# modelscope/FunCodec

Measured on AMD Instinct MI355X. Metric: audio-seconds encoded+decoded per wall-sec, 16k-nq32ds640, higher is better.
Workload: dtype f32; 1 GPU; BASELINE.json configs[1]: encodec 16k-nq32ds640 (57.6M, synthetic seeded checkpoint), run_mod=inference (encode + 32-stage RVQ + decode), 16 x 10 s utterances per GPU in micro-batches of 16, n_q=32; utterances_per_gpu=16, samples_per_utterance=160000, micro_batch=16, global_utterances=16, ranks_seen=1, parallelism=single GPU

## Files before the change

funcodec_amd/_lib.py:

```python
from __future__ import annotations

import ctypes as C
import os

from . import build as _build

FC_MAX_RATIOS = 8
FC_ABI_VERSION = 7


class FcArch(C.Structure):
    _fields_ = [
        ("abi_version", C.c_int32), ("sample_rate", C.c_int32), ("audio_normalize", C.c_int32),
        ("n_filters", C.c_int32), ("dimension", C.c_int32), ("n_ratios", C.c_int32),
        ("ratios", C.c_int32 * FC_MAX_RATIOS),
        ("kernel_size", C.c_int32), ("last_kernel_size", C.c_int32), ("residual_kernel_size", C.c_int32),
        ("compress", C.c_int32), ("lstm_layers", C.c_int32), ("lstm_skip", C.c_int32),
        ("elu_alpha", C.c_float), ("gn_eps", C.c_float),
        ("codebook_size", C.c_int32), ("num_quantizers", C.c_int32),
        ("norm_type", C.c_int32), ("causal", C.c_int32), ("n_residual_layers", C.c_int32), ("dilation_base", C.c_int32),
        ("model_type", C.c_int32), ("input_channels", C.c_int32), ("n_fft", C.c_int32), ("stft_hop", C.c_int32),
        ("ratios_f", C.c_int32 * FC_MAX_RATIOS),
        ("enc_conv_group_ratio", C.c_int32), ("dec_conv_group_ratio", C.c_int32), ("dec_tr_conv_group_ratio", C.c_int32),
        ("codec_dim", C.c_int32), ("codec_range", C.c_float),
        ("q0_ds_ratio", C.c_int32),
        ("seq_model", C.c_int32), ("seq_heads", C.c_int32), ("seq_ff", C.c_int32),
    ]


class FcWork(C.Structure):
    _fields_ = [("total_flops", C.c_double), ("total_bytes", C.c_double), ("conv_flops", C.c_double),
                ("conv_bytes", C.c_double), ("lstm_flops", C.c_double), ("rvq_flops", C.c_double),
                ("conv_launches", C.c_int32), ("total_launches", C.c_int32)]


class FcProf(C.Structure):
    _fields_ = [("kernel", C.c_char * 64), ("total_ms", C.c_double), ("flops", C.c_double), ("bytes", C.c_double),
                ("launches", C.c_int32), ("reserved", C.c_int32)]


FC_PROF_CLASSES = 48


class FcLauraStack(C.Structure):
    _fields_ = [("idim", C.c_int32), ("d_model", C.c_int32), ("heads", C.c_int32), ("ff", C.c_int32), ("layers", C.c_int32),
                ("act", C.c_int32), ("embed_relu", C.c_int32), ("norm_style", C.c_int32)]


class FcLauraArch(C.Structure):
    _fields_ = [("abi_version", C.c_int32), ("input_size", C.c_int32), ("vocab_size", C.c_int32), ("codebook_size", C.c_int32),
                ("codebook_dim", C.c_int32), ("num_quantizers", C.c_int32), ("predict_nq", C.c_int32), ("pos_emb_split", C.c_int32),
                ("bidirectional_inputs", C.c_int32), ("max_positions", C.c_int32),
                ("text_encoder", FcLauraStack), ("codec_lm", FcLauraStack), ("codec_encoder", FcLauraStack)]


_P = C.c_void_p
SYMBOLS = {
    "fc_abi_version": (C.c_int, []),
    "fc_last_error": (C.c_char_p, []),
    "fc_engine_create": (C.c_int, [C.POINTER(FcArch), C.c_int, C.POINTER(_P)]),
    "fc_engine_destroy": (None, [_P]),
    "fc_engine_num_weights": (C.c_int, [_P]),
    "fc_engine_weight_info": (C.c_int, [_P, C.c_int, C.POINTER(C.c_char_p), C.POINTER(C.c_int64)]),
    "fc_engine_set_weight": (C.c_int, [_P, C.c_char_p, _P, C.POINTER(C.c_int64), C.c_int]),
    "fc_engine_finalize": (C.c_int, [_P]),
    "fc_engine_hop_length": (C.c_int, [_P]),
    "fc_engine_frames": (C.c_int, [_P, C.c_int]),
    "fc_engine_decoded_samples": (C.c_int, [_P, C.c_int]),
    "fc_engine_workspace_bytes": (C.c_size_t, [_P, C.c_int, C.c_int]),
    "fc_encode": (C.c_int, [_P, _P, C.c_int, C.c_int, C.c_int, _P, _P, _P, _P, _P, _P, C.c_size_t, _P]),
    "fc_decode_emb": (C.c_int, [_P, _P, _P, C.c_int, C.c_int, C.c_int, _P, _P, C.c_size_t, _P]),
    "fc_decode_codes": (C.c_int, [_P, _P, C.c_int, C.c_int, C.c_int, C.c_int, _P, _P, _P, C.c_size_t, _P]),
    "fc_encode_decode": (C.c_int, [_P, _P, C.c_int, C.c_int, C.c_int, C.c_int, _P, _P, _P, _P, _P, _P, C.c_size_t, _P]),
    "fc_ragged_workspace_bytes": (C.c_size_t, [_P, C.c_int, C.c_int]),
    "fc_encode_ragged": (C.c_int, [_P, _P, _P, C.c_int, C.c_int, C.c_int, _P, _P, _P, _P, _P, _P, C.c_size_t, _P]),
    "fc_decode_emb_ragged": (C.c_int, [_P, _P, _P, _P, C.c_int, C.c_int, C.c_int, _P, _P, C.c_size_t, _P]),
    "fc_decode_codes_ragged": (C.c_int, [_P, _P, _P, C.c_int, C.c_int, C.c_int, C.c_int, _P, _P, _P, C.c_size_t, _P]),
    "fc_encode_decode_ragged": (C.c_int, [_P, _P, _P, C.c_int, C.c_int, C.c_int, C.c_int, _P, _P, _P, _P, _P, _P, C.c_size_t, _P]),
    "fc_engine_set_row_nq": (C.c_int, [_P, _P, C.c_int, _P]),
    "fc_rvq_encode": (C.c_int, [_P, _P, C.c_int, C.c_int, _P, _P, _P, C.c_size_t, _P]),
    "fc_q0_source_frames": (C.c_int, [C.c_int, _P]),
    "fc_layer_forward": (C.c_int, [_P, C.c_char_p, _P, C.c_int, C.c_int, C.c_int, _P, _P, C.c_size_t, _P]),
    "fc_layer_forward_src": (C.c_int, [_P, C.c_char_p, _P, _P, _P, _P, _P, C.c_int, C.c_int, C.c_int, _P, _P, C.c_size_t, _P]),
    "fc_layer_out_len": (C.c_int, [_P, C.c_char_p, C.c_int]),
    "fc_layer2d_forward": (C.c_int, [_P, C.c_char_p, _P, _P, _P, _P, C.c_int, C.c_int, C.c_int, C.c_int, C.c_int, _P, _P, C.c_size_t, _P]),
    "fc_layer2d_out_shape": (C.c_int, [_P, C.c_char_p, C.c_int, C.c_int, C.c_int, C.c_int, C.POINTER(C.c_int64)]),
    "fc_freq_synthesis": (C.c_int, [_P, _P, _P, _P, C.c_int, C.c_int, C.c_int, C.c_int, C.c_int, _P, _P, _P, C.c_size_t, _P]),
    "fc_freq_synthesis_size": (C.c_int, [_P, C.c_int, C.c_int, C.c_int, C.c_int, C.c_int, C.POINTER(C.c_size_t)]),
    "fc_lstm_forward": (C.c_int, [_P, C.c_char_p, _P, C.c_int, C.c_int, _P, _P, C.c_size_t, _P]),
    "fc_seq_forward": (C.c_int, [_P, C.c_char_p, _P, C.c_int, C.c_int, _P, _P, C.c_size_t, _P]),
    "fc_resblock_forward": (C.c_int, [_P, C.c_char_p, _P, C.c_int, C.c_int, _P, _P, C.c_size_t, _P]),
    "fc_resblock_forward_src": (C.c_int, [_P, C.c_char_p, _P, _P, _P, _P, C.c_int, C.c_int, _P, _P, C.c_size_t, _P]),
    "fc_engine_work": (C.c_int, [_P, C.c_int, C.c_int, C.c_int, C.POINTER(FcWork)]),
    "fc_engine_profile": (C.c_int, [_P, C.c_int]),
    "fc_engine_profile_read": (C.c_int, [_P, C.POINTER(FcProf)]),
    "fc_debug_timeline": (C.c_int, [_P]),
    "fc_debug_conv_layout": (C.c_int, [C.c_int] * 7 + [_P, _P, C.c_size_t, _P, C.c_size_t]),
    "fc_debug_freq_features": (C.c_int, [_P, C.c_size_t, C.c_int]),
    "fc_codec_json_bound": (C.c_size_t, [C.c_int, C.c_int]),
    "fc_format_codec_json": (C.c_int, [_P, C.c_int, C.c_int, C.c_int, C.c_int, C.c_int, _P, C.c_size_t, C.POINTER(C.c_size_t)]),
    "fc_write_wav_pcm16": (C.c_int, [C.c_char_p, _P, C.c_int, C.c_int, C.c_int]),
    "fc_overlap_add": (C.c_int, [_P, _P, C.c_int, C.c_int, C.c_int, C.c_int, C.c_int, _P, _P]),
    "fc_engine_status": (C.c_int, [_P, C.POINTER(C.c_uint)]),
    "fc_stream_state_bytes": (C.c_size_t, [_P, C.c_int]),
    "fc_stream_create": (C.c_int, [_P, C.c_int, C.c_int, C.c_int, _P, C.c_size_t, C.POINTER(_P)]),
    "fc_stream_destroy": (None, [_P]),
    "fc_stream_min_first": (C.c_int, [_P, C.c_int]),
    "fc_stream_workspace_bytes": (C.c_size_t, [_P]),
    "fc_stream_reset": (C.c_int, [_P, _P, _P]),
    "fc_stream_encode": (C.c_int, [_P, _P, C.c_int, C.c_int, _P, _P, _P, C.POINTER(C.c_int), _P, C.c_size_t, _P]),
    "fc_stream_decode_codes": (C.c_int, [_P, _P, C.c_int, C.c_int, _P, _P, _P, C.c_size_t, _P]),
    "fc_stream_decode_emb": (C.c_int, [_P, _P, C.c_int, C.c_int, _P, _P, C.c_size_t, _P]),
    "fc_stream_lstm_forward": (C.c_int, [_P, C.c_int, _P, C.c_int, _P, _P, C.c_size_t, _P]),
    "fc_seqstream_state_bytes": (C.c_size_t, [_P, C.c_int, C.c_int]),
    "fc_seqstream_create": (C.c_int, [_P, C.c_int, C.c_int, C.c_int, C.c_int, _P, C.c_size_t, C.POINTER(_P)]),
    "fc_seqstream_forward": (C.c_int, [_P, C.c_int, _P, C.c_int, _P, _P, C.c_size_t, _P]),
    "fc_slots_state_bytes": (C.c_size_t, [_P, C.c_int]),
    "fc_slots_create": (C.c_int, [_P, C.c_int, C.c_int, C.c_int, _P, C.c_size_t, C.POINTER(_P)]),
    "fc_slots_destroy": (None, [_P]),
    "fc_slots_min_first": (C.c_int, [_P, C.c_int]),
    "fc_slots_workspace_bytes": (C.c_size_t, [_P]),
    "fc_slots_encode": (C.c_int, [_P, _P, C.c_int, _P, _P, _P, _P, _P, _P, _P, C.c_size_t, _P]),
    "fc_slots_decode_codes": (C.c_int, [_P, _P, C.c_int, _P, _P, C.c_int, _P, _P, _P, C.c_size_t, _P]),
    "fc_slots_decode_emb": (C.c_int, [_P, _P, C.c_int, _P, _P, C.c_int, _P, _P, C.c_size_t, _P]),
    "fc_slots_lstm_forward": (C.c_int, [_P, C.c_int, _P, C.c_int, _P, _P, _P, _P, C.c_size_t, _P]),
    "fc_seqslots_state_bytes": (C.c_size_t, [_P, C.c_int, C.c_int]),
    "fc_seqslots_create": (C.c_int, [_P, C.c_int, C.c_int, C.c_int, C.c_int, _P, C.c_size_t, C.POINTER(_P)]),
    "fc_seqslots_forward": (C.c_int, [_P, C.c_int, _P, C.c_int, _P, _P, _P, _P, C.c_size_t, _P]),
    "fc_graphstream_set": (C.c_int, [_P, C.c_int]),
    "fc_graphstream_enabled": (C.c_int, [_P]),
    "fc_graphstream_counts": (C.c_int, [_P, C.POINTER(C.c_int64)]),
    "fc_graphslots_set": (C.c_int, [_P, C.c_int]),
    "fc_graphslots_enabled": (C.c_int, [_P]),
    "fc_graphslots_counts": (C.c_int, [_P, C.POINTER(C.c_int64)]),
    "fc_laura_create": (C.c_int, [C.POINTER(FcLauraArch), C.c_int, C.POINTER(_P)]),
    "fc_laura_destroy": (None, [_P]),
    "fc_laura_num_weights": (C.c_int, [_P]),
    "fc_laura_weight_info": (C.c_int, [_P, C.c_int, C.POINTER(C.c_char_p), C.POINTER(C.c_int64)]),
    "fc_laura_set_weight": (C.c_int, [_P, C.c_char_p, _P, C.POINTER(C.c_int64), C.c_int]),
    "fc_laura_finalize": (C.c_int, [_P]),
    "fc_laura_workspace_bytes": (C.c_size_t, [_P, C.c_int, C.c_int, C.c_int, C.c_int]),
    "fc_laura_encode": (C.c_int, [_P, _P, _P, _P, C.c_int, C.c_int, _P, _P, C.c_size_t, _P]),
    "fc_laura_lm_logprobs": (C.c_int, [_P, _P, _P, C.c_int, C.c_int, _P, _P, C.c_int, _P, C.c_int, _P, C.c_size_t, _P]),
    "fc_laura_decode_codec": (C.c_int, [_P, _P, _P, C.c_int, C.c_int, _P, _P, C.c_int, C.c_int, C.c_int, C.c_int, C.c_float,
                                        C.c_uint64, _P, _P, _P, _P, _P, C.c_size_t, _P]),
    "fc_laura_codec_emb": (C.c_int, [_P, _P, _P, C.c_int, C.c_int, _P, C.c_int, _P, C.c_int, _P, _P, C.c_size_t, _P]),
    "fc_laura_linear": (C.c_int, [_P, C.c_char_p, _P, C.c_int, C.c_int, C.c_int, _P, _P, C.c_size_t, _P]),
    "fc_laura_debug_probe": (C.c_int, [_P, C.c_size_t, C.c_int, C.c_int, C.c_int]),
    "fc_laura_set_persistent_step": (C.c_int, [_P, C.c_int]),
    "fc_laura_persistent_step_fallbacks": (C.c_int, [_P]),
    "fc_laura_slots_state_bytes": (C.c_size_t, [_P, C.c_int, C.c_int, C.c_int]),
    "fc_laura_slots_create": (C.c_int, [_P, C.c_int, C.c_int, C.c_int, _P, C.c_size_t, C.POINTER(_P)]),
    "fc_laura_slots_destroy": (None, [_P]),
    "fc_laura_slots_workspace_bytes": (C.c_size_t, [_P, C.c_int, C.c_int]),
    "fc_laura_slots_start": (C.c_int, [_P, C.c_int, _P, C.c_int, _P, C.c_int, C.c_int, C.c_int, C.c_int, C.c_float, C.c_uint64, _P,
                                       _P, C.c_size_t, _P]),
    "fc_laura_slots_step": (C.c_int, [_P, C.c_int, _P, _P, _P]),
    "fc_laura_slots_take": (C.c_int, [_P, C.c_int, _P, C.c_int, _P, _P]),
    "fc_laura_slots_start_from": (C.c_int, [_P, C.c_int, C.c_int, C.c_int, C.c_int, C.c_int, C.c_float, C.c_uint64, _P, _P]),
    "fc_laura_slots_fork": (C.c_int, [_P, C.c_int, C.c_int, C.c_int, C.c_int, C.c_int, C.c_int, C.c_float, C.c_uint64, _P]),
    "fc_laura_slots_state_bytes_scored": (C.c_size_t, [_P, C.c_int, C.c_int, C.c_int, C.c_int]),
    "fc_laura_slots_create_scored": (C.c_int, [_P, C.c_int, C.c_int, C.c_int, C.c_int, _P, C.c_size_t, C.POINTER(_P)]),
    "fc_laura_slots_score": (C.c_int, [_P, C.c_int, _P, C.c_int, C.POINTER(C.c_int32), C.POINTER(C.c_int32)]),
    "fc_laura_slots_set_rules": (C.c_int, [_P, C.c_int, C.c_float, C.c_int, C.c_float, C.c_int, C.c_int]),
    "fc_laura_slots_start_many_workspace_bytes": (C.c_size_t, [_P, C.c_int, C.c_int, C.c_int]),
    "fc_laura_slots_start_many": (C.c_int, [_P, C.c_int, _P, _P, _P, C.c_int, _P, _P, C.c_int, _P, _P, _P, _P, _P, _P, C.c_size_t, _P]),
    "fc_laura_slots_start_from_session": (C.c_int, [_P, C.c_int, _P, C.c_int, C.c_int, C.c_int, C.c_int, C.c_float, C.c_uint64, _P, _P]),
    "fc_laura_slots_state_bytes_wide": (C.c_size_t, [_P, C.c_int, C.c_int, C.c_int, C.c_int]),
    "fc_laura_slots_create_wide": (C.c_int, [_P, C.c_int, C.c_int, C.c_int, C.c_int, _P, C.c_size_t, C.POINTER(_P)]),
    "fc_laura_slots_state_bytes_queued": (C.c_size_t, [_P, C.c_int, C.c_int, C.c_int, C.c_int]),
    "fc_laura_slots_create_queued": (C.c_int, [_P, C.c_int, C.c_int, C.c_int, C.c_int, _P, _P, C.c_size_t, C.POINTER(_P)]),
    "fc_laura_slots_submit": (C.c_int, [_P, C.c_int, C.c_int, C.c_int, C.c_int, C.c_float, C.c_uint64, C.c_float, C.c_int, C.c_float, C.c_int,
                                        C.c_int, C.POINTER(C.c_int32), _P]),
    "fc_laura_slots_queue_status": (C.c_int, [_P, C.POINTER(C.c_int64), C.POINTER(C.c_int64), C.POINTER(C.c_int64), C.POINTER(C.c_int64),
                                              C.POINTER(C.c_int64), _P]),
# ... 34 lines not shown
```

funcodec_amd/csrc/engine.hip:

```cpp
#include <hip/hip_runtime.h>

#include <algorithm>
#include <array>
#include <cmath>
#include <cstdio>
#include <cstring>
#include <map>
#include <memory>
#include <string>
#include <vector>

#include "../../include/funcodec_amd.h"
#include "kernels.h"
#include "laura_kernels.h"
#include "ragged_kernels.h"
#include "seq_kernels.h"
#include "slots_kernels.h"
#include "stream_kernels.h"

namespace {

thread_local std::string g_err;

int fail(const std::string& msg) { g_err = msg; return 1; }
// ... 40 lines not shown
    float *wt = nullptr, *bias = nullptr, *gamma = nullptr, *beta = nullptr;
    int* koff = nullptr;
};

struct LstmLayer {
    ConvLayer inproj;
    float* whh = nullptr;
    float* wcat = nullptr;
    float* bperm = nullptr;
};

struct LstmBlock {
    std::string prefix;
    int H = 0;
    std::vector<LstmLayer> layers;
};

struct TfLayer {
    ConvLayer qkv;
    ConvLayer out, ff1, ff2;
    float *n1g = nullptr, *n1b = nullptr, *n2g = nullptr, *n2b = nullptr;
};

struct TfBlock {
    std::string prefix;
    int C = 0, heads = 4, ff = 2048;
    std::vector<TfLayer> layers;
    float *ag = nullptr, *ab = nullptr;
};

struct Act {
    float* raw = nullptr;
    float* aff = nullptr;
    int C = 0, T = 0;
    bool normed = false;
    int ld = 0;
};

int ceil_div_i(int a, int b) { return (a + b - 1) / b; }

const char* kLstmPersistClass = "lstm_persist_kernel<NS> (whole recurrence of one SLSTM block, one launch)";
const char* kLstmWaveClass = "lstm_wave_kernel<NS> (whole recurrence of one SLSTM block: T + L - 1 launches incl. gaps)";
const char* kRvqClass = "rvq_encode_kernel<D, RS> (all stages of the residual quantiser)";

}

struct fc_engine {
    fc_arch arch;
    int device = 0;
    bool finalized = false;
    std::vector<std::pair<std::string, std::vector<int64_t>>> expected;
    std::map<std::string, HostTensor> host;
    ConvLayer enc_first, enc_last, dec_first, dec_last;
    struct ResBlock {
        ConvLayer shortcut, block1, block3;
        bool fused_head = false;
        float *wsc = nullptr, *wb1 = nullptr;
        float *bsc = nullptr, *bb1 = nullptr;
    };
    struct Stage { std::vector<ResBlock> res; ConvLayer resample; };
    std::vector<Stage> enc_stages, dec_stages;
    LstmBlock enc_lstm, dec_lstm;
    TfBlock enc_tf, dec_tf;
    std::map<std::string, TfBlock*> tf_by_prefix;
    std::map<std::string, ConvLayer*> by_prefix;
    std::map<std::string, ResBlock*> res_by_prefix;
    ConvLayer enc2_first, dec2_last, stft, istft;
    ConvLayer q_in, q_out;
    bool q_proj = false;
    int cdim() const { return q_proj ? arch.codec_dim : arch.dimension; }
    int audio_ch() const { return arch.model_type == 0 && arch.input_channels == 2 ? 2 : 1; }
    std::vector<std::vector<ConvLayer>> dec_up_phases;
    int halo2 = 3;
    float* win2 = nullptr;
    std::map<std::string, LstmBlock*> lstm_by_prefix;
    float *cb = nullptr, *enorm = nullptr;
    float* cb_frag = nullptr;
    std::vector<void*> dev_allocs;
    volatile unsigned* status_host = nullptr;
    unsigned* status_dev = nullptr;
    std::vector<int32_t> row_nq;
    int* row_nq_dev = nullptr;
    size_t row_nq_cap = 0;
    bool lstm_persist_ok = true;
    int persist_checked_B = -1; bool persist_checked_val = false;
    bool profiling = false;
    struct Span { hipEvent_t a, b; int cls; double flops, bytes; };
    std::vector<Span> spans;
    std::vector<hipEvent_t> event_pool;
    size_t events_used = 0;
    std::vector<std::string> prof_names;
    int prof_class(const std::string& name) {
        for (size_t i = 0; i < prof_names.size(); ++i)
            if (prof_names[i] == name) return (int)i;
        if ((int)prof_names.size() >= FC_PROF_CLASSES) return FC_PROF_CLASSES - 1;
        prof_names.push_back(name);
        return (int)prof_names.size() - 1;
    }
};

struct Session {
    fc_engine* e = nullptr;
    int B = 0, max_chunk = 0, n_q = 0;
    float* state = nullptr;
    size_t state_floats = 0;
    std::map<const ConvLayer*, size_t> carry;
    size_t enc_lstm_off = 0, dec_lstm_off = 0;
    int max_frames = 0;
    size_t enc_kv_off = 0, dec_kv_off = 0;
    size_t carried_floats = 0;
    int enc_min_first = 0, dec_min_first = 0;
    std::vector<float> ones;

    struct GraphKey {
        int form = 0;
        int width = 0, parity = 0, n_q = 0, use_scale = 0;
        std::array<const void*, 5> ptr{};
        const void* ws = nullptr; size_t ws_bytes = 0;
        const void* stream = nullptr;
        const void* nq_table = nullptr; int nq_rows = 0;
        bool operator==(const GraphKey& o) const {
            return form == o.form && width == o.width && parity == o.parity && n_q == o.n_q && use_scale == o.use_scale && ptr == o.ptr && ws == o.ws &&
                   ws_bytes == o.ws_bytes && stream == o.stream && nq_table == o.nq_table && nq_rows == o.nq_rows;
        }
    };
    struct Graph { GraphKey key; hipGraphExec_t exec = nullptr; unsigned long long used = 0; };
    static constexpr size_t kMaxGraphs = 16;
    bool graph_on = false;
    std::vector<Graph> graphs;
    unsigned long long graph_tick = 0;
    int64_t graph_counts[4] = {0, 0, 0, 0};
    void drop_graphs() {
        for (Graph& g : graphs) (void)hipGraphExecDestroy(g.exec);
        graphs.clear();
    }
    Session() = default;
    Session(const Session&) = delete;
    Session& operator=(const Session&) = delete;
    ~Session() { drop_graphs(); }
};

struct fc_stream : Session {
    int enc_pushes = 0, dec_pushes = 0;
    int enc_frames = 0, dec_frames = 0;
    bool enc_done = false;
    bool broken = false;
};

struct fc_slots : Session {
    enum Phase : char { Idle, Running, Ended, Poisoned };
    std::vector<char> enc_phase, dec_phase;
    int enc_pushes = 0, dec_pushes = 0;
    std::vector<int32_t> push;
    std::vector<int32_t> enc_frames, dec_frames;
};

namespace {

hipEvent_t prof_event(fc_engine* e) {
    if (e->events_used == e->event_pool.size()) {
        hipEvent_t ev;
        if (hipEventCreate(&ev) != hipSuccess) return nullptr;
        e->event_pool.push_back(ev);
    }
    return e->event_pool[e->events_used++];
}
// ... 530 lines not shown
    if (upload(e, fc::conv_koff_table(L.gk, L.gstride, L.dil, L.CC, L.BN, L.row ? 1 : 0), &L.koff)) return 1;
    return 0;
}

int pack_conv(fc_engine* e, ConvLayer& L) {
    const std::string inner = L.transposed ? ".convtr" : ".conv";
    std::vector<float> folded;
    if (L.wnorm) {
        const auto& V = e->host[L.prefix + inner + ".weight_v"].data;
        const auto& G = e->host[L.prefix + inner + ".weight_g"].data;
        const size_t d0 = L.transposed ? L.cin : L.cout, inner_n = V.size() / d0;
        folded.resize(V.size());
        for (size_t r = 0; r < d0; ++r) {
            double ss = 0.0;
            for (size_t j = 0; j < inner_n; ++j) ss += (double)V[r * inner_n + j] * (double)V[r * inner_n + j];
            const float nrm = (float)sqrt(ss);
            const float sc = G[r] / nrm;
            for (size_t j = 0; j < inner_n; ++j) folded[r * inner_n + j] = V[r * inner_n + j] * sc;
        }
    }
    const auto& W = L.wnorm ? folded : e->host[L.prefix + inner + ".weight"].data;
    const auto& Bv = e->host[L.prefix + inner + ".bias"].data;
    if (!L.transposed) {
        if (pack_gemm(e, L, W, Bv)) return 1;
        if (L.cout == 1 && L.stride == 1) {
            if (upload(e, W, &L.w_plain)) return 1;
            L.bias0 = Bv[0];
        }
    } else {
        const int r = L.stride;
        if (L.k != 2 * r) return fail("ConvTranspose1d with kernel != 2*stride is not supported: " + L.prefix);
        std::vector<float> wg((size_t)L.M * L.cin * 2), bg(L.M);
        for (int co = 0; co < L.cout; ++co)
            for (int p = 0; p < r; ++p) {
                const int m = co * r + p;
                bg[m] = Bv[co];
                for (int ci = 0; ci < L.cin; ++ci) {
                    wg[((size_t)m * L.cin + ci) * 2 + 0] = W[((size_t)ci * L.cout + co) * L.k + p + r];
                    wg[((size_t)m * L.cin + ci) * 2 + 1] = W[((size_t)ci * L.cout + co) * L.k + p];
                }
            }
        if (pack_gemm(e, L, wg, bg)) return 1;
    }
    if (L.has_norm) {
        if (upload(e, e->host[L.prefix + ".norm.weight"].data, &L.gamma)) return 1;
        if (upload(e, e->host[L.prefix + ".norm.bias"].data, &L.beta)) return 1;
    }
    return 0;
}

std::vector<float> folded_conv_weight(fc_engine* e, const ConvLayer& L) {
    const std::string inner = L.transposed ? ".convtr" : ".conv";
    if (!L.wnorm) return e->host[L.prefix + inner + ".weight"].data;
    const auto& V = e->host[L.prefix + inner + ".weight_v"].data;
    const auto& G = e->host[L.prefix + inner + ".weight_g"].data;
    const size_t d0 = L.transposed ? L.cin : L.cout, inner_n = V.size() / d0;
    std::vector<float> folded(V.size());
    for (size_t r = 0; r < d0; ++r) {
        double ss = 0.0;
        for (size_t j = 0; j < inner_n; ++j) ss += (double)V[r * inner_n + j] * (double)V[r * inner_n + j];
        const float sc = G[r] / (float)sqrt(ss);
        for (size_t j = 0; j < inner_n; ++j) folded[r * inner_n + j] = V[r * inner_n + j] * sc;
    }
    return folded;
}

int pack_reshead(fc_engine* e, fc_engine::ResBlock& R) {
    static const int enable = fc::ab_knob("FC_RESHEAD", 1);
    const int C = R.shortcut.cin, hid = R.block1.cout, K = R.block1.k;
    R.fused_head = enable && R.shortcut.cout == C && R.block1.cin == C && fc::reshead_ok(C, hid, R.shortcut.k, K, R.block1.dil, R.block1.stride) &&
                   R.shortcut.has_norm == R.block1.has_norm;
    if (!R.fused_head) return 0;
    const std::vector<float> Wsc = folded_conv_weight(e, R.shortcut), Wb1 = folded_conv_weight(e, R.block1);
    std::vector<float> a((size_t)C * C), b((size_t)K * C * hid);
    for (int m = 0; m < C; ++m)
        for (int c = 0; c < C; ++c) a[(size_t)c * C + m] = Wsc[(size_t)m * C + c];
    for (int h = 0; h < hid; ++h)
        for (int c = 0; c < C; ++c)
            for (int kk = 0; kk < K; ++kk) b[((size_t)kk * C + c) * hid + h] = Wb1[((size_t)h * C + c) * K + kk];
    if (upload(e, a, &R.wsc) || upload(e, b, &R.wb1)) return 1;
    if (upload(e, e->host[R.shortcut.prefix + ".conv.bias"].data, &R.bsc)) return 1;
    if (upload(e, e->host[R.block1.prefix + ".conv.bias"].data, &R.bb1)) return 1;
    return 0;
}


int pack_conv2d(fc_engine* e, ConvLayer& L) {
    const std::vector<float> W = folded_weight_nd(e, L.prefix + ".conv", L.wnorm, (size_t)L.cout);
    const auto& Bv = e->host[L.prefix + ".conv.bias"].data;
    const int C = L.c2d, kf = L.kf, kt = L.k;
    const int cpg = C / L.groups, opg = L.cout / L.groups;
    std::vector<float> wg((size_t)L.cout * kf * C * kt, 0.f);
    for (int m = 0; m < L.cout; ++m)
        for (int cl = 0; cl < cpg; ++cl) {
            const int ci = (m / opg) * cpg + cl;
            for (int a = 0; a < kf; ++a)
                for (int b = 0; b < kt; ++b)
                    wg[((size_t)m * (kf * C) + (size_t)a * C + ci) * kt + b] = W[(((size_t)m * cpg + cl) * kf + a) * kt + b];
        }
    if (pack_gemm(e, L, wg, Bv)) return 1;
    static const int gconv_env = fc::ab_knob("FC_GCONV", 1);
    if (gconv_env && L.groups > 1 && L.dil == 1 && fc::gconv2d_ok(cpg, opg, kf, kt, L.stride) && upload(e, W, &L.w_group)) return 1;
    if (L.cout <= 4 && L.stride == 1 && L.sf == 1 && (L.k == 3 || L.k == 5 || L.k == 7) && upload(e, wg, &L.w_plain)) return 1;
    if (L.has_norm) {
        if (upload(e, e->host[L.prefix + ".norm.weight"].data, &L.gamma)) return 1;
        if (upload(e, e->host[L.prefix + ".norm.bias"].data, &L.beta)) return 1;
    }
    return 0;
}

int pack_convtr2d(fc_engine* e, const ConvLayer& S, std::vector<ConvLayer>& phases) {
    const std::vector<float> W = folded_weight_nd(e, S.prefix + ".convtr", S.wnorm, (size_t)S.c2d);
    const auto& Bv = e->host[S.prefix + ".convtr.bias"].data;
    const int C = S.c2d, cout = S.cout, kf = S.kf, kt = S.k, sf = S.sf, r = S.stride;
    const int cpg = C / S.groups, opg = cout / S.groups;
    for (int p = 0; p < sf; ++p) {
        ConvLayer& L = phases[p];
        std::vector<float> wg((size_t)L.M * L.cin * 2, 0.f), bg(L.M);
        for (int co = 0; co < cout; ++co)
            for (int ph = 0; ph < r; ++ph) {
                const int m = co * r + ph;
                bg[m] = Bv[co];
                for (int rr = 0; rr < 2; ++rr)
                    for (int ci = (co / opg) * cpg; ci < (co / opg + 1) * cpg; ++ci) {
                        const int a = p + (1 - rr) * sf;
                        const float* w = &W[(((size_t)ci * opg + co % opg) * kf + a) * kt];
                        const size_t c1 = (size_t)rr * C + ci;
                        wg[((size_t)m * L.cin + c1) * 2 + 0] = w[ph + r];
                        wg[((size_t)m * L.cin + c1) * 2 + 1] = w[ph];
                    }
            }
        if (pack_gemm(e, L, wg, bg)) return 1;
    }
    ConvLayer& L0 = phases[0];
    static const int gconv_env = fc::ab_knob("FC_GCONV", 1);
    if (gconv_env && S.groups > 1 && fc::gconvtr2d_ok(cpg, opg, r)) {
        if (upload(e, W, &L0.w_group) || upload(e, Bv, &L0.w_plain)) return 1;
    }
    if (S.has_norm) {
        if (upload(e, e->host[S.prefix + ".norm.weight"].data, &L0.gamma)) return 1;
        if (upload(e, e->host[S.prefix + ".norm.bias"].data, &L0.beta)) return 1;
    }
    return 0;
}

int pack_dft(fc_engine* e) {
    const int N = e->arch.n_fft, hop = e->arch.stft_hop, F = N / 2 + 1, taps = ceil_div_i(N, hop);
    std::vector<double> win(N);
    for (int n = 0; n < N; ++n) win[n] = 0.5 - 0.5 * cos(2.0 * M_PI * n / N);
    auto tw_cos = [&](long long k) { k %= N; return (k % (N / 2)) == N / 4 ? 0.0 : cos(2.0 * M_PI * (double)k / N); };
    auto tw_sin = [&](long long k) { k %= N; return (k % (N / 2)) == 0 ? 0.0 : sin(2.0 * M_PI * (double)k / N); };
    {
        ConvLayer& L = e->stft;
        std::vector<float> wg((size_t)2 * F * hop * taps, 0.f), bg(2 * F, 0.f);
        for (int f = 0; f < F; ++f)
            for (int j = 0; j < hop; ++j)
                for (int a = 0; a < taps; ++a) {
                    const int n = a * hop + j;
                    if (n >= N) continue;
                    const long long k = (long long)f * n;
                    wg[((size_t)f * hop + j) * taps + a] = (float)(win[n] * tw_cos(k));
                    wg[((size_t)(F + f) * hop + j) * taps + a] = tw_sin(k) == 0.0 ? 0.f : (float)(-win[n] * tw_sin(k));
                }
        if (pack_gemm(e, L, wg, bg)) return 1;
    }
    {
// ... 266 lines not shown
    y.C = C; y.T = T;
    y.raw = cx.alloc<float>((size_t)B * C * T);
    float* part = kv ? cx.alloc<float>(fc::seq_attn_cached_part_floats(B, tb.heads, DK)) : nullptr;
    fc::SeqRows rows;
    double row_pairs = 0.0, row_keys = 0.0;
    if (kv && kv->rows) {
        rows.len = kv->len; rows.pos = kv->pos_dev; rows.S = B; rows.T = T; rows.F = kv->F;
        for (int b = 0; b < B && kv->host_len; ++b) {
            const int len = kv->host_len[b], n = len > 0 ? fc::ragged_cols(len, rows.len.div, rows.len.mul, rows.len.add) : 0, pos = kv->host_pos[b];
            if (n < 1) continue;
            if (n > T || pos < 0 || pos + n > kv->F) { cx.fail("internal: a slot's frames leave the chunk or the key / value cache"); return y; }
            rows.max_waves = std::max(rows.max_waves, fc::seq_attn_rows_waves(n, pos));
            row_pairs += (double)n * pos + 0.5 * (double)n * (n + 1);
            row_keys += pos + n;
        }
        if (kv->grid_bound) rows.max_waves = (T + 15) / 16 * fc::kSeqCachedMaxUnits;
    }
    const double pairs = tb.layers.empty() ? 0.0
                         : kv && kv->rows ? row_pairs / B
                         : kv ? (double)T * kv->pos + 0.5 * (double)T * (T + 1)
                              : (e->arch.causal ? 0.5 * (double)T * (T + 1) : (double)T * T);
    const double attn_fl = 4.0 * B * pairs * C;
    cx.attn_flops += attn_fl * tb.layers.size();
    const char* pre = tb.prefix.c_str();
    auto ln = [&](const float* add, const float* g, const float* b, float* out) {
        cx.launch("transformer LayerNorm", pre, [] { return "layernorm_fm_kernel (transformer, residual add fused)"; }, 0.0, 4.0 * B * C * T * (add ? 4 : 2),
                  [&] { return fc::laura::launch_layernorm_fm(x, add, add ? x : nullptr, g, b, 1e-12f, 0, 1.f, out, B, C, T, cx.st); });
    };
    cx.launch("combine", pre, [&] { return fc::launch_combine(src_of(in), fc::Src(), 0, 1.f, nullptr, B, C, T, T, x, sC, T, 1, cx.st); });
    fc::Src sxn; sxn.ptr = xn; sxn.used = 1;
    fc::Src sctx; sctx.ptr = ctx; sctx.used = 1;
    fc::Src shb; shb.ptr = hb; shb.used = 1;
    const float* pending = nullptr;
    size_t block = 0;
    for (const TfLayer& L : tb.layers) {
        ln(pending, L.n1g, L.n1b, xn);
        run_conv(e, cx, L.qkv, sxn, fc::Src(), 0, T, qkv, 3 * sC, T, 1);
        if (kv && kv->rows) {
            const size_t plane = (size_t)B * C * kv->F;
            float* kc = kv->base ? kv->base + 2 * plane * block : nullptr;
            fc::SeqCacheAppendRows ap;
            ap.qkv = qkv; ap.kc = kc; ap.vc = kc ? kc + plane : nullptr; ap.C = C; ap.rows = rows;
            cx.launch("transformer cache append", pre, [] { return "seq_cache_append_rows_kernel (slot push: K and V of every row into its cache)"; }, 0.0,
                      4.0 * B * 4.0 * C * T, [&] { return fc::launch_seq_cache_append_rows(ap, cx.st); });
            fc::SeqAttnRows a;
            a.qkv = qkv; a.kc = ap.kc; a.vc = ap.vc; a.out = ctx; a.part = part; a.H = tb.heads; a.DK = DK; a.rows = rows;
            cx.launch("transformer cached attention", pre, [&] { return fc::seq_attn_rows_kernel_name(DK); }, attn_fl,
                      4.0 * C * (2.0 * B * T + 2.0 * row_keys), [&] { return fc::launch_seq_attn_rows(a, cx.st); });
        } else if (kv) {
            const size_t plane = (size_t)B * C * kv->F;
            float* kc = kv->base ? kv->base + 2 * plane * block : nullptr;
            fc::SeqCacheAppend ap;
            ap.qkv = qkv; ap.kc = kc; ap.vc = kc ? kc + plane : nullptr; ap.B = B; ap.C = C; ap.n = T; ap.pos = kv->pos; ap.F = kv->F;
            cx.launch("transformer cache append", pre, [] { return "seq_cache_append_kernel (streaming: K and V of a push into the cache)"; }, 0.0,
                      4.0 * B * 4.0 * C * T, [&] { return fc::launch_seq_cache_append(ap, cx.st); });
            fc::SeqAttnCached a;
            a.qkv = qkv; a.kc = ap.kc; a.vc = ap.vc; a.out = ctx; a.part = part; a.B = B; a.H = tb.heads; a.DK = DK; a.n = T; a.pos = kv->pos; a.F = kv->F;
            cx.launch("transformer cached attention", pre, [&] { return fc::seq_attn_cached_kernel_name(DK); }, attn_fl,
                      4.0 * B * C * (2.0 * T + 2.0 * (kv->pos + T)), [&] { return fc::launch_seq_attn_cached(a, cx.st); });
        } else {
            fc::SeqAttn a;
            a.qkv = qkv; a.out = ctx; a.B = B; a.H = tb.heads; a.DK = DK; a.T = T; a.causal = e->arch.causal ? 1 : 0;
            cx.launch("transformer attention", pre, [&] { return fc::seq_attn_kernel_name(DK); }, attn_fl, 4.0 * B * 4.0 * C * T,
                      [&] { return fc::launch_seq_attn(a, cx.st); });
        }
        ++block;
        run_conv(e, cx, L.out, sctx, fc::Src(), 0, T, dl, sC, T, 1);
        ln(dl, L.n2g, L.n2b, xn);
        run_conv(e, cx, L.ff1, sxn, fc::Src(), 0, T, hb, (long long)ff * T, T, 1);
        cx.launch("ReLU", pre, [] { return "act_kernel (transformer feed-forward ReLU)"; }, 0.0, 8.0 * B * ff * T,
                  [&] { return fc::laura::launch_act(hb, (size_t)B * ff * T, 1, cx.st); });
        run_conv(e, cx, L.ff2, shb, fc::Src(), 0, T, dl, sC, T, 1);
        pending = dl;
    }
    ln(pending, tb.ag, tb.ab, y.raw);
    return y;
}

bool has_seq(const LstmBlock& lb, const TfBlock& tb) { return lb.H != 0 || tb.C != 0; }
Act run_seq(fc_engine* e, Ctx& cx, const LstmBlock& lb, const TfBlock& tb, const Act& in, int T) {
    return tb.C ? run_transformer(e, cx, tb, in, T) : run_lstm(e, cx, lb, in, T);
}

void run_reshead(fc_engine* e, Ctx& cx, const fc_engine::ResBlock& R, fc::Src a0, fc::Src a1, int T, Act* sc, Act* b1) {
    const int C = R.shortcut.cin, hid = R.block1.cout;
    const ConvGeom g = conv_geom(R.block1, T);
    sc->C = C; sc->T = T; b1->C = hid; b1->T = T;
    sc->raw = cx.alloc<float>((size_t)cx.B * C * T);
    b1->raw = cx.alloc<float>((size_t)cx.B * hid * T);
    fc::ResHeadLaunch c;
    c.s0 = a0; c.s1 = a1; c.wsc = R.wsc; c.wb1 = R.wb1; c.bsc = R.bsc; c.bb1 = R.bb1;
    c.out_sc = sc->raw; c.out_b1 = b1->raw;
    c.B = cx.B; c.C = C; c.T = T; c.k = R.block1.k; c.dil = R.block1.dil; c.padL = g.padL; c.padR = g.padR;
    c.alpha = e->arch.elu_alpha;
    const int nblk = fc::reshead_ntiles(T);
    if (R.shortcut.has_norm) {
        c.part_sc = cx.alloc<double>((size_t)cx.B * nblk * 2);
        c.part_b1 = cx.alloc<double>((size_t)cx.B * nblk * 2);
        sc->aff = cx.alloc<float>((size_t)cx.B * C * 2); sc->normed = true;
        b1->aff = cx.alloc<float>((size_t)cx.B * hid * 2); b1->normed = true;
    }
    const double fl = 2.0 * cx.B * (double)T * ((double)C * C + (double)hid * C * R.block1.k);
    const double by = 4.0 * cx.B * (double)T * ((double)C * (a1.used ? 2 : 1) + C + hid);
    cx.conv_flops += fl; cx.conv_bytes += by;
    auto cls = [&] {
        char nm[64];
        snprintf(nm, sizeof(nm), "reshead_kernel<%d, %d, %s>", C, R.block1.k, a1.used ? "true" : "false");
        return std::string(nm);
    };
    cx.conv_launch("fused res-block head", R.shortcut.prefix.c_str(), cls, fl, by, [&] { return fc::launch_reshead(c, cx.st); });
    conv_finish(e, cx, R.shortcut, c.part_sc, nblk, (double)C * T, sc->aff);
    conv_finish(e, cx, R.block1, c.part_b1, nblk, (double)hid * T, b1->aff);
}

struct Pass {
    enum Kind { Offline, Stream, Ragged, Slots } kind = Offline;
    const Session* sess = nullptr;
    int n = 0;
    bool final = false;
    const int* lengths = nullptr;
    int frame_div = 1;
    const int* flags = nullptr;
    const int32_t* host_push = nullptr;
    const int* pos = nullptr;
    bool graphed = false;
};

inline fc::RagLen ragged_len(const Ctx& cx, const Pass& p) {
    fc::RagLen r;
    r.lens = p.lengths;
    if (cx.dec_side) { r.div = p.frame_div; r.mul = cx.rate; }
    else r.div = cx.rate;
    return r;
}

Act ragged_conv(fc_engine* e, Ctx& cx, const Pass& p, const ConvLayer& L, fc::Src s0, fc::Src s1, int elu, int T);
Act stream_conv(fc_engine* e, Ctx& cx, const Pass& p, const ConvLayer& L, fc::Src s0, fc::Src s1, int elu, int Tc);
Act slots_conv(fc_engine* e, Ctx& cx, const Pass& p, const ConvLayer& L, fc::Src s0, fc::Src s1, int elu, int T);
float* lstm_state(const Session& s, bool dec);
TfCache tf_cache(const Session& s, bool dec, int pos);

Act walk_conv(fc_engine* e, Ctx& cx, const Pass& p, Role role, const ConvLayer& L, fc::Src s0, fc::Src s1, int elu, int T) {
    switch (p.kind) {
        case Pass::Stream: if (carries_context(role)) return stream_conv(e, cx, p, L, s0, s1, elu, T); break;
        case Pass::Slots: if (carries_context(role)) return slots_conv(e, cx, p, L, s0, s1, elu, T); break;
        case Pass::Ragged: if (L.k > 1 || L.has_norm) return ragged_conv(e, cx, p, L, s0, s1, elu, T); break;
        case Pass::Offline: break;
    }
    return run_conv(e, cx, L, s0, s1, elu, T);
}

void run_bottleneck(fc_engine* e, Ctx& cx, const Pass& p, bool dec, const Act& x, fc::Src* a0, fc::Src* a1) {
    const LstmBlock& lb = dec ? e->dec_lstm : e->enc_lstm;
    const TfBlock& tb = dec ? e->dec_tf : e->enc_tf;
    *a0 = src_of(x); *a1 = fc::Src();
    if (!has_seq(lb, tb)) return;
    Act y;
    switch (p.kind) {
        case Pass::Stream:
            if (tb.C) {
                const TfCache kv = tf_cache(*p.sess, dec, dec ? static_cast<const fc_stream*>(p.sess)->dec_frames : static_cast<const fc_stream*>(p.sess)->enc_frames);
                if (!cx.dry && kv.pos + x.T > p.sess->max_frames) { cx.fail("internal: a push past max_frames reached the transformer"); return; }
                y = run_transformer(e, cx, tb, x, x.T, &kv);
            } else {
                y = run_lstm(e, cx, lb, x, x.T, lstm_state(*p.sess, dec));
            }
            break;
        case Pass::Slots: {
            const fc::RagLen steps = ragged_len(cx, p);
            if (tb.C) {
                TfCache kv = tf_cache(*p.sess, dec, 0);
                kv.rows = true; kv.len = steps; kv.pos_dev = p.pos;
                if (p.host_push) { kv.host_len = p.host_push; kv.host_pos = p.host_push + 2 * cx.B; }
                kv.grid_bound = p.graphed;
                y = run_transformer(e, cx, tb, x, x.T, &kv);
            } else {
                y = run_lstm(e, cx, lb, x, x.T, lstm_state(*p.sess, dec), &steps);
            }
            break;
        }
        case Pass::Ragged:
        case Pass::Offline: y = run_seq(e, cx, lb, tb, x, x.T); break;
    }
    *a0 = src_of(y);
    if (e->arch.lstm_skip) *a1 = src_of(x);
}

void run_resblocks(fc_engine* e, Ctx& cx, const Pass& p, const fc_engine::Stage& S, fc::Src a0, fc::Src a1, int T, Act* sc, Act* b3) {
    for (const auto& R : S.res) {
        Act b1;
        if (p.kind == Pass::Offline && R.fused_head && !a0.div) {
            run_reshead(e, cx, R, a0, a1, T, sc, &b1);
        } else {
            *sc = walk_conv(e, cx, p, Role::Shortcut, R.shortcut, a0, a1, 0, T);
            b1 = walk_conv(e, cx, p, Role::Block1, R.block1, a0, a1, 1, T);
        }
        *b3 = walk_conv(e, cx, p, Role::Block3, R.block3, src_of(b1), fc::Src(), 1, b1.T);
        a0 = src_of(*sc); a1 = src_of(*b3);
    }
}

Act run_encoder(fc_engine* e, Ctx& cx, const Pass& p, fc::Src wav, int T) {
    cx.dec_side = false; cx.rate = 1; cx.no_xq = p.kind == Pass::Ragged;
    Act x = walk_conv(e, cx, p, Role::First, e->enc_first, wav, fc::Src(), 0, T);
    for (auto& S : e->enc_stages) {
        Act sc, b3;
        run_resblocks(e, cx, p, S, src_of(x), fc::Src(), x.T, &sc, &b3);
        x = walk_conv(e, cx, p, Role::Resample, S.resample, src_of(sc), src_of(b3), 1, sc.T);
        cx.rate *= S.resample.stride;
    }
    fc::Src a0, a1;
    run_bottleneck(e, cx, p, false, x, &a0, &a1);
    return walk_conv(e, cx, p, Role::Last, e->enc_last, a0, a1, 1, x.T);
}

Act run_decoder(fc_engine* e, Ctx& cx, const Pass& p, const float* z_bdt, int Tf) {
    fc::Src s; s.ptr = z_bdt; s.used = 1;
    cx.dec_side = true; cx.rate = 1; cx.no_xq = p.kind == Pass::Ragged;
    Act x = walk_conv(e, cx, p, Role::First, e->dec_first, s, fc::Src(), 0, Tf);
    fc::Src a0, a1;
    run_bottleneck(e, cx, p, true, x, &a0, &a1);
    int T = Tf;
    for (auto& S : e->dec_stages) {
        Act up = walk_conv(e, cx, p, Role::Resample, S.resample, a0, a1, 1, T);
        cx.rate *= S.resample.stride;
        Act sc, b3;
        run_resblocks(e, cx, p, S, src_of(up), fc::Src(), up.T, &sc, &b3);
        a0 = src_of(sc); a1 = src_of(b3);
        T = up.T;
    }
    return walk_conv(e, cx, p, Role::Last, e->dec_last, a0, a1, 1, T);
}



Act2 materialise2d(fc_engine* e, Ctx& cx, const ConvLayer& L, const Act2& x0, const Act2* x1, int elu, int pad) {
    const int B = cx.B, C = L.c2d;
    Act2 m;
    m.C = C; m.F = x0.F; m.T = x0.T; m.halo = x0.halo;
    m.buf = cx.alloc<float>((size_t)B * (m.F + 2 * m.halo) * C * m.T);
    const bool fuse_halo = !pad && halo_fuse_on() && m.F > m.halo;
    cx.launch("combine2d", L.prefix.c_str(), [&] {
        if (x0.halo < pad) return hipErrorInvalidValue;
        return fc::launch_combine2d(x0.buf, x0.aff, x0.halo, x1 ? x1->buf : nullptr, x1 ? x1->aff : nullptr, x1 ? x1->halo : 0, elu, e->arch.elu_alpha,
                                    B, m.F, C, m.T, m.buf, m.halo, cx.st, fuse_halo ? 1 : 0);
    });
    if (pad) cx.launch("halo rows", L.prefix.c_str(), [&] { return fc::launch_halo_rows_short(m.buf, B, m.F, m.halo, pad, C, m.T, cx.st); });
    else if (!fuse_halo) cx.launch("halo rows", L.prefix.c_str(), [&] { return fc::launch_halo_rows(m.buf, B, m.F, m.halo, C, m.T, 0, cx.st); });
    return m;
}

Act2 run_conv2d(fc_engine* e, Ctx& cx, const ConvLayer& L, Act2 x0, const Act2* x1, int elu, int out_halo) {
    const int B = cx.B, C = L.c2d, kf = L.kf, sf = L.sf;
    const int tot_f = (kf - 1) - (sf - 1), f_after = tot_f / 2, f_before = tot_f - f_after;
    const int Fo = (x0.F + tot_f - kf) / sf + 1;
    const ConvGeom g = conv_geom(L, x0.T);
    const int fpad = std::max(f_before, f_after);
    if (x0.F <= fpad) { x0 = materialise2d(e, cx, L, x0, x1, elu, fpad); x1 = nullptr; elu = 0; }
    bool mat;
    if (L.w_group) {
        static const int gmat = fc::ab_knob("FC_GCONV_MAT", 1);
        mat = gmat && kf >= 4 && x1;
    } else {
        static const int few_mat = fc::ab_knob("FC_FEWOUT_MAT", 1);
        const bool few_out = few_mat && L.cout <= 4 && L.stride == 1 && sf == 1 && (L.k == 3 || L.k == 5 || L.k == 7) && kf > 1;
        mat = (L.Mpad / L.BM >= 3 || few_out || L.force_plain) && (x0.normed || x1 || elu);
    }
    if (mat) { x0 = materialise2d(e, cx, L, x0, x1, elu, 0); x1 = nullptr; elu = 0; }
    Act2 o;
    o.C = L.cout; o.F = Fo; o.T = g.Tout; o.halo = out_halo;
    o.buf = cx.alloc<float>((size_t)B * (Fo + 2 * out_halo) * L.cout * g.Tout);
    if (!cx.dry && (x0.halo < f_before || x0.halo < f_after || (x1 && x1->halo != x0.halo))) {
        cx.fail("internal: frequency halo too small for " + L.prefix);
        return o;
    }
    const long long rowsz = (long long)C * x0.T, orow = (long long)L.cout * g.Tout;
    const double by = 4.0 * B * ((double)C * x0.F * x0.T * (x1 ? 2 : 1) + (double)L.cout * Fo * g.Tout);
    o.normed = L.has_norm;
    if (L.w_group) {
        fc::GConvLaunch c;
        c.src0 = at(x0.buf, (x0.halo - f_before) * rowsz); c.aff0 = x0.aff;
        if (x1) { c.src1 = at(x1->buf, (x1->halo - f_before) * rowsz); c.aff1 = x1->aff; }
        c.w = L.w_group; c.bias = L.bias;
        c.out = at(o.buf, out_halo * orow);
        c.B = B; c.C = C; c.M = L.cout; c.G = L.groups; c.Tin = x0.T; c.Tout = g.Tout; c.Fo = Fo; c.kf = kf; c.kt = L.k; c.sf = sf; c.st = L.stride;
        c.padL = g.padL; c.padR = g.padR; c.elu = elu; c.alpha = e->arch.elu_alpha;
        c.guard_lo = cx.base; c.guard_hi = cx.base ? cx.base + cx.cap : nullptr;
        c.in_sB = (long long)(x0.F + 2 * x0.halo) * rowsz; c.in_sF = rowsz;
        c.out_sB = (long long)(Fo + 2 * out_halo) * orow; c.out_sF = orow;
        const bool fuse_halo = halo_fuse_on() && fc::gconv2d_fuses_halo(kf, L.k, L.stride, Fo, out_halo);
// ... 841 lines not shown
void slots_advance(fc_slots* Q, bool decode, const int32_t* counts, const int32_t* flags, int whole) {
    if (Q->max_frames <= 0) return;
    std::vector<int32_t>& frames = decode ? Q->dec_frames : Q->enc_frames;
    for (int b = 0; b < Q->B; ++b)
        if (counts[b] > 0) frames[b] = ((flags[b] & FC_SLOT_START) ? 0 : frames[b]) + ceil_div_i(counts[b], whole);
}

void slots_commit(fc_slots* Q, bool decode, const int32_t* counts, const int32_t* flags, bool ok) {
    std::vector<char>& phase = decode ? Q->dec_phase : Q->enc_phase;
    if (!ok) {
        std::fill(Q->enc_phase.begin(), Q->enc_phase.end(), (char)fc_slots::Poisoned);
        std::fill(Q->dec_phase.begin(), Q->dec_phase.end(), (char)fc_slots::Poisoned);
        return;
    }
    for (int b = 0; b < Q->B; ++b)
        if (counts[b] > 0) phase[b] = (flags[b] & FC_SLOT_FINAL) ? fc_slots::Ended : fc_slots::Running;
    slots_advance(Q, decode, counts, flags, decode ? 1 : total_hop(Q->e));
    ++(decode ? Q->dec_pushes : Q->enc_pushes);
}

}

extern "C" {

int fc_abi_version(void) { return FC_ABI_VERSION; }
const char* fc_last_error(void) { return g_err.c_str(); }
void fc_set_last_error_(const char* msg) { g_err = msg ? msg : ""; }

int fc_engine_create(const fc_arch* arch, int device, fc_engine** out) {
    if (!arch || !out) return fail("null argument");
    if (arch->abi_version != FC_ABI_VERSION) return fail("fc_arch.abi_version mismatch");
    if (arch->n_residual_layers < 1 || arch->n_residual_layers > 8 || arch->dilation_base < 1)
        return fail("fc_arch.n_residual_layers must be in 1..8 and dilation_base >= 1");
    if (arch->norm_type < 0 || arch->norm_type > 2) return fail("fc_arch.norm_type must be 0 (GroupNorm), 1 (weight_norm) or 2 (none)");
    if (arch->norm_type == 0 && arch->causal) return fail("GroupNorm convs cannot be causal (the reference refuses it too, conv.py:46-47)");
    if (arch->n_ratios < 1 || arch->n_ratios > FC_MAX_RATIOS) return fail("n_ratios out of range");
    if (arch->compress < 1 || arch->n_filters < 2 || (arch->n_filters % arch->compress) != 0) return fail("bad n_filters/compress");
    if (arch->n_filters % 2) return fail("n_filters must be even");
    const int D = arch->dimension;
    if (!(D == 16 || D == 32 || D == 64 || D == 128 || D == 256 || D == 512)) return fail("dimension must be one of 16/32/64/128/256/512");
    if (arch->codec_dim < 0 || arch->codec_range < 0.f) return fail("fc_arch.codec_dim / codec_range must be >= 0");
    if (arch->codec_dim > 0) {
        const int Dc = arch->codec_dim;
        if (!(Dc == 16 || Dc == 32 || Dc == 64 || Dc == 128 || Dc == 256 || Dc == 512)) return fail("codec_dim must be one of 16/32/64/128/256/512");
    }
    if (arch->codebook_size % 64 || (arch->codebook_size > 128 && arch->codebook_size % 128))
        return fail("codebook_size must be a multiple of 64, and of 128 above 128 (8 waves x 16-code tiles)");
    if (arch->seq_model != 0 && arch->seq_model != 1) return fail("fc_arch.seq_model must be 0 (SLSTM) or 1 (TransformerEncoder)");
    if (arch->seq_model == 0 && arch->lstm_layers > 0 && ((arch->n_filters << arch->n_ratios) % 16)) return fail("LSTM width must be a multiple of 16");
    if (arch->seq_model == 0 && arch->lstm_layers > FC_LSTM_MAX_LAYERS) return fail("too many LSTM layers");
    if (arch->seq_model == 1 && arch->lstm_layers > 0) {
        const int C = arch->n_filters << arch->n_ratios;
        if (arch->seq_heads < 1 || C % arch->seq_heads || !fc::seq_attn_supported(C / arch->seq_heads))
            return fail("transformer bottleneck: head size C / seq_heads must be 16, 32, 64, 128 or 256 (C = " + std::to_string(C) + ")");
        if (C % 16 || C > 1024) return fail("transformer bottleneck: width must be a multiple of 16 and at most 1024 (LayerNorm kernel)");
        if (arch->seq_ff < 1) return fail("transformer bottleneck: seq_ff must be >= 1");
        if (arch->lstm_layers > 64) return fail("transformer bottleneck: at most 64 blocks");
    }
    for (int i = 0; i < arch->n_ratios; ++i)
        if (arch->ratios[i] < 1) return fail("ratios must be >= 1");
    if (arch->model_type != 0 && arch->model_type != 1) return fail("fc_arch.model_type must be 0 (encodec) or 1 (freq_codec, mag_phase)");
    if (arch->model_type == 0 && (arch->input_channels < 0 || arch->input_channels > 2))
        return fail("encodec: input_channels must be 1 (0 reads as 1) or 2 (stereo; the reference asserts channels <= 2, codec_basic.py:344)");
    if (arch->model_type == 1) {
        if (arch->norm_type != 0 && arch->norm_type != 1) return fail("freq_codec: norm must be time_group_norm or weight_norm");
        if (arch->input_channels != 3 && arch->input_channels != 2)
            return fail("freq_codec: input_channels must be 3 (codec_domain mag_phase: log-magnitude, phase re, phase im) or 2 (mag_angle: log-magnitude, angle)");
        if (arch->n_fft < 64 || (arch->n_fft & (arch->n_fft - 1)) || arch->stft_hop < 1 || arch->stft_hop > arch->n_fft)
            return fail("freq_codec: n_fft must be a power of two >= 64 and 1 <= stft_hop <= n_fft");
        if (arch->stft_hop % 2) return fail("freq_codec: stft_hop must be even");
        if (arch->dilation_base != 1 && arch->n_residual_layers > 1) return fail("freq_codec: dilated residual stacks are not built for the 2-D nets");
        int f = arch->n_fft / 2 + 1;
        for (int i = arch->n_ratios - 1; i >= 0; --i) {
            const int fr = arch->ratios_f[i];
            if (fr < 1) return fail("freq_codec: ratios_f must be >= 1");
            const int tot = (2 * fr - 1) - (fr - 1);
            f = (f + tot - 2 * fr) / fr + 1;
        }
        if (f != 1) return fail("freq_codec: the frequency ratios must reduce n_fft / 2 + 1 bins to exactly one");
    }
    fc_engine* e = new fc_engine();
    e->arch = *arch;
    e->device = device;
    build_plan(e);
    for (const auto& kv : e->by_prefix)
        if (kv.second->unsupported) {
            const std::string msg = "stride " + std::to_string(kv.second->gstride) + " / kernel " + std::to_string(kv.second->gk) + " of " + kv.first +
                                    " exceeds the conv kernel's slab (ratios above 16 are not built)";
            delete e;
            return fail(msg);
        }
    if (arch->model_type == 1) {
        std::vector<const ConvLayer*> ls;
        for (auto* st : {&e->enc_stages, &e->dec_stages})
            for (auto& S : *st) {
                for (auto& R : S.res) { ls.push_back(&R.shortcut); ls.push_back(&R.block1); ls.push_back(&R.block3); }
                ls.push_back(&S.resample);
            }
        for (const ConvLayer* L : ls)
            if (L->groups < 1 || L->c2d % L->groups || L->cout % L->groups) {
                const std::string msg = "freq_codec: conv_group_ratio gives " + std::to_string(L->groups) + " groups for " + L->prefix + " (" +
                                        std::to_string(L->c2d) + " -> " + std::to_string(L->cout) + " channels)";
                delete e;
                return fail(msg);
            }
    }
    *out = e;
    return 0;
}

int fc_engine_profile(fc_engine* e, int enable) {
    if (!e) return fail("null engine");
    e->profiling = enable != 0;
    return 0;
}

int fc_engine_profile_read(fc_engine* e, fc_prof* out) {
    if (!e || !out) return fail("null argument");
    for (int i = 0; i < FC_PROF_CLASSES; ++i) {
        memset(&out[i], 0, sizeof(fc_prof));
        if (i < (int)e->prof_names.size()) strncpy(out[i].kernel, e->prof_names[i].c_str(), sizeof(out[i].kernel) - 1);
    }
    if (!e->spans.empty()) HIP_TRY(hipEventSynchronize(e->spans.back().b));
    for (auto& s : e->spans) {
        float ms = 0.f;
        if (hipEventElapsedTime(&ms, s.a, s.b) != hipSuccess) continue;
        out[s.cls].total_ms += ms; out[s.cls].flops += s.flops; out[s.cls].bytes += s.bytes; out[s.cls].launches += 1;
    }
    e->spans.clear();
    e->events_used = 0;
    return 0;
}

void fc_engine_destroy(fc_engine* e) {
    if (!e) return;
    for (hipEvent_t ev : e->event_pool) (void)hipEventDestroy(ev);
    for (void* p : e->dev_allocs) (void)hipFree(p);
    if (e->status_host) (void)hipHostFree((void*)e->status_host);
    delete e;
}

int fc_engine_num_weights(const fc_engine* e) { return e ? (int)e->expected.size() : 0; }

int fc_engine_weight_info(const fc_engine* e, int i, const char** name, int64_t* dims) {
    if (!e || i < 0 || i >= (int)e->expected.size()) return -1;
    if (name) *name = e->expected[i].first.c_str();
    const auto& d = e->expected[i].second;
    if (dims) for (size_t j = 0; j < d.size(); ++j) dims[j] = d[j];
    return (int)d.size();
}

int fc_engine_set_weight(fc_engine* e, const char* name, const float* host, const int64_t* dims, int ndim) {
    if (!e || !name || !host || !dims) return fail("null argument");
    if (e->finalized) return fail("engine already finalized");
    for (auto& ex : e->expected) {
        if (ex.first != name) continue;
        if ((int)ex.second.size() != ndim) return fail(std::string("rank mismatch for ") + name);
        size_t n = 1;
        for (int j = 0; j < ndim; ++j) {
            if (ex.second[j] != dims[j]) return fail(std::string("shape mismatch for ") + name);
            n *= (size_t)dims[j];
        }
        HostTensor& t = e->host[name];
        t.dims.assign(dims, dims + ndim);
        t.data.assign(host, host + n);
        t.set = true;
        return 0;
    }
    g_err = std::string("tensor not part of the hot path: ") + name;
    return 2;
}

int fc_engine_finalize(fc_engine* e) {
    if (!e) return fail("null engine");
    if (e->finalized) return 0;
    for (auto& ex : e->expected)
        if (!e->host.count(ex.first) || !e->host[ex.first].set) return fail("checkpoint is missing tensor " + ex.first);
    int ndev = 0;
    if (hipGetDeviceCount(&ndev) != hipSuccess || ndev <= 0)
        return fail("no HIP device visible: the FunCodec MI355X engine has no CPU fallback");
    HIP_TRY(hipSetDevice(e->device));
    hipDeviceProp_t prop;
    HIP_TRY(hipGetDeviceProperties(&prop, e->device));
    if (std::string(prop.gcnArchName).find("gfx950") == std::string::npos)
        return fail(std::string("device is ") + prop.gcnArchName + ", this library is built for gfx950 only");
    if (e->arch.model_type == 1) {
        if (pack_conv2d(e, e->enc2_first) || pack_conv2d(e, e->dec2_last)) return 1;
        for (auto& S : e->enc_stages) {
            for (auto& R : S.res)
                if (pack_conv2d(e, R.shortcut) || pack_conv2d(e, R.block1) || pack_conv2d(e, R.block3)) return 1;
            if (pack_conv2d(e, S.resample)) return 1;
        }
        for (size_t si = 0; si < e->dec_stages.size(); ++si) {
            auto& S = e->dec_stages[si];
            for (auto& R : S.res)
                if (pack_conv2d(e, R.shortcut) || pack_conv2d(e, R.block1) || pack_conv2d(e, R.block3)) return 1;
            if (pack_convtr2d(e, S.resample, e->dec_up_phases[si])) return 1;
        }
        if (pack_conv(e, e->enc_last) || pack_conv(e, e->dec_first)) return 1;
        if (pack_dft(e)) return 1;
    } else {
        int err = 0;
        for_each_conv(e, [&](const ConvVisit& v) { if (!err && v.role == Role::Shortcut) err = pack_reshead(e, *v.block); });
        for_each_conv(e, [&](const ConvVisit& v) { if (!err) err = pack_conv(e, v.L); });
        if (err) return 1;
    }
    if (pack_lstm(e, e->enc_lstm)) return 1;
    if (pack_lstm(e, e->dec_lstm)) return 1;
    if (pack_tf(e, e->enc_tf) || pack_tf(e, e->dec_tf)) return 1;
    const auto& E = e->host["quantizer.rq.model.embed"].data;
    const int nq = e->arch.num_quantizers, K = e->arch.codebook_size, D = e->cdim();
    if (e->q_proj) {
        if (pack_gemm(e, e->q_in, e->host["quantizer.input_proj.weight"].data, e->host["quantizer.input_proj.bias"].data)) return 1;
        if (pack_gemm(e, e->q_out, e->host["quantizer.output_proj.weight"].data, e->host["quantizer.output_proj.bias"].data)) return 1;
    }
    std::vector<float> en((size_t)nq * K);
    for (size_t r = 0; r < (size_t)nq * K; ++r) {
        volatile float s = 0.f;
        for (int d = 0; d < D; ++d) {
            volatile float sq = E[r * D + d] * E[r * D + d];
            s = s + sq;
        }
        en[r] = s;
    }
    if (upload(e, E, &e->cb)) return 1;
    if (K % 16 == 0 && D % 16 == 0) {
        std::vector<float> F((size_t)nq * K * D);
        for (int i = 0; i < nq; ++i)
            for (int c = 0; c < K; ++c)
                for (int d = 0; d < D; ++d) {
                    const size_t tile = (size_t)i * (K / 16) + c / 16;
                    F[((tile * (D / 16) + d / 16) * 4 + (d % 16) / 4) * 64 + (size_t)(c % 16) * 4 + d % 4] = E[((size_t)i * K + c) * D + d];
                }
        if (upload(e, F, &e->cb_frag)) return 1;
    }
    if (upload(e, en, &e->enorm)) return 1;
    {
        void* hp = nullptr;
        HIP_TRY(hipHostMalloc(&hp, FC_STATUS_WORDS * sizeof(unsigned), hipHostMallocMapped));
        memset(hp, 0, FC_STATUS_WORDS * sizeof(unsigned));
        void* dp = nullptr;
        HIP_TRY(hipHostGetDevicePointer(&dp, hp, 0));
        e->status_host = (volatile unsigned*)hp;
        e->status_dev = (unsigned*)dp;
    }
    e->host.clear();
    HIP_TRY(hipDeviceSynchronize());
    e->finalized = true;
    return 0;
}

int fc_engine_hop_length(const fc_engine* e) { return e ? total_hop(e) : 0; }
int fc_engine_frames(const fc_engine* e, int n_samples) { return e ? frames_for(e, n_samples) : 0; }
int fc_engine_decoded_samples(const fc_engine* e, int n_frames) { return e ? decoded_samples(e, n_frames) : 0; }

size_t fc_engine_workspace_bytes(const fc_engine* ce, int B, int T) {
    fc_engine* e = const_cast<fc_engine*>(ce);
    if (!e || B <= 0 || T <= 0) return 0;
    const int Tf = frames_for(e, T), D = e->arch.dimension;
    Ctx cx = dry_ctx(e, B);
    float* q = nullptr;
    do_encode(e, cx, nullptr, T, e->arch.num_quantizers, nullptr, nullptr, nullptr, nullptr, nullptr, &q);
    cx.alloc<float>((size_t)B * Tf * D);
    cx.alloc<float>((size_t)B * Tf * D);
    decoder_input_emb(e, cx, nullptr, Tf);
    do_decode(e, cx, nullptr, Tf, nullptr, decoded_samples(e, Tf), nullptr);
    return cx.off + 4096;
}

int fc_engine_work(const fc_engine* ce, int B, int T, int n_q, fc_work* out) {
    fc_engine* e = const_cast<fc_engine*>(ce);
    if (!e || !out) return fail("null argument");
    Ctx cx = dry_ctx(e, B);
    float* q = nullptr;
    float quantized_mark;
    do_encode(e, cx, nullptr, T, n_q, nullptr, &quantized_mark, nullptr, nullptr, nullptr, &q);
    do_decode(e, cx, nullptr, frames_for(e, T), nullptr, T, nullptr);
    out->conv_flops = cx.conv_flops; out->conv_bytes = cx.conv_bytes;
    out->lstm_flops = cx.lstm_flops; out->rvq_flops = cx.rvq_flops;
    out->total_flops = cx.conv_flops + cx.lstm_flops + cx.rvq_flops + cx.attn_flops;
    out->total_bytes = cx.conv_bytes;
    out->conv_launches = cx.conv_launches; out->total_launches = cx.launches;
    return 0;
}

namespace {
struct FeatHookDisarm { ~FeatHookDisarm() { g_feat_hook = FeatHook(); } };
}
// ... 288 lines not shown
    run_synthesis_2d(e, cx, last, scale, out_len, wav, &spec);
    if (spec_out)
        cx.launch("copy", "spectrum", [&] { return hipMemcpyAsync(spec_out, spec, (size_t)B * 2 * F * Tp * sizeof(float), hipMemcpyDeviceToDevice, cx.st); });
    return cx.err;
}
}

int fc_freq_synthesis_size(const fc_engine* ce, int B, int C, int F, int Tp, int out_len, size_t* workspace_bytes) {
    fc_engine* e = const_cast<fc_engine*>(ce);
    if (freq_synthesis_check(e, B, C, F, Tp, out_len)) return 1;
    if (!workspace_bytes) return fail("null argument");
    Ctx cx = dry_ctx(e, B);
    if (freq_synthesis(e, cx, nullptr, nullptr, nullptr, Tp, out_len, nullptr, nullptr)) return 1;
    *workspace_bytes = cx.off + 4096;
    return 0;
}

int fc_freq_synthesis(fc_engine* e, const float* dec, const float* aff, const float* scale, int B, int C, int F, int Tp, int out_len, float* wav,
                      float* spec, void* workspace, size_t workspace_bytes, void* stream) {
    if (freq_synthesis_check(e, B, C, F, Tp, out_len)) return 1;
    if (!dec || !wav) return fail("bad argument");
    if (check_ready(e)) return 1;
    Ctx cx = make_ctx(e, B, workspace, workspace_bytes, stream);
    return freq_synthesis(e, cx, dec, aff, scale, Tp, out_len, wav, spec);
}

namespace {
fc::Src hook_src(const float* x, const float* aff, const float* div) {
    fc::Src s;
    s.ptr = x; s.aff = aff; s.div = div;
    s.used = x ? ((aff || div) ? 3 : 1) : 0;
    return s;
}
}

static int layer_src_check(const fc_engine* e, const char* prefix, const float* x0, const float* aff0, const float* div0, const float* x1,
                           const float* aff1, int B, int T, const ConvLayer** out) {
    if (!e || !prefix || !x0 || B <= 0 || T <= 0 || (aff1 && !x1) || (aff0 && div0)) return fail("bad argument");
    auto it = e->by_prefix.find(prefix);
    if (it == e->by_prefix.end()) return fail(std::string("unknown layer ") + prefix);
    const ConvLayer& L = *it->second;
    if (L.c2d > 0)
        return fail(std::string("layer ") + prefix + " is a 2-D layer of the STFT-domain codec: use fc_layer2d_forward");
    if (x1 && !L.dual) return fail("fc_layer_forward_src: " + L.prefix + " is planned for one source (its staging has no room for two)");
    if (div0 && &L != &e->enc_first) return fail("fc_layer_forward_src: div0 is the encoder's first conv's volume scale (" + e->enc_first.prefix + ")");
    *out = &L;
    return 0;
}

int fc_layer_forward_src(fc_engine* e, const char* prefix, const float* x0, const float* aff0, const float* div0, const float* x1,
                         const float* aff1, int B, int T, int apply_elu, float* y, void* workspace, size_t workspace_bytes, void* stream) {
    const ConvLayer* L = nullptr;
    if (layer_src_check(e, prefix, x0, aff0, div0, x1, aff1, B, T, &L)) return 1;
    if (!y) return fail("bad argument");
    if (check_ready(e)) return 1;
    Ctx cx = make_ctx(e, B, workspace, workspace_bytes, stream);
    Act o = run_conv(e, cx, *L, hook_src(x0, aff0, div0), hook_src(x1, aff1, nullptr), apply_elu, T);
    if (cx.err) return 1;
    HIP_TRY(fc::launch_combine(src_of(o), fc::Src(), 0, 1.f, nullptr, B, o.C, o.T, o.T, y, (long long)o.C * o.T, o.T, 1, cx.st));
    return 0;
}

int fc_layer_forward(fc_engine* e, const char* prefix, const float* x, int B, int T, int apply_elu, float* y,
                     void* workspace, size_t workspace_bytes, void* stream) {
    return fc_layer_forward_src(e, prefix, x, nullptr, nullptr, nullptr, nullptr, B, T, apply_elu, y, workspace, workspace_bytes, stream);
}

int fc_resblock_forward_src(fc_engine* e, const char* prefix, const float* x0, const float* aff0, const float* x1, const float* aff1, int B,
                            int T, float* y, void* workspace, size_t workspace_bytes, void* stream) {
    if (!e || !prefix || !x0 || !y || B <= 0 || T <= 0 || (aff1 && !x1)) return fail("bad argument");
    auto it = e->res_by_prefix.find(prefix);
    if (it == e->res_by_prefix.end()) return fail(std::string("unknown residual block ") + prefix);
    const fc_engine::ResBlock& R = *it->second;
    if (x1 && !R.shortcut.dual)
        return fail(std::string("fc_resblock_forward_src: block ") + prefix + " is planned for one source (its staging has no room for two)");
    if (check_ready(e)) return 1;
    Ctx cx = make_ctx(e, B, workspace, workspace_bytes, stream);
    fc_engine::Stage one;
    one.res.push_back(R);
    Act sc, b3;
    run_resblocks(e, cx, Pass(), one, hook_src(x0, aff0, nullptr), hook_src(x1, aff1, nullptr), T, &sc, &b3);
    if (cx.err) return 1;
    HIP_TRY(fc::launch_combine(src_of(sc), src_of(b3), 0, 1.f, nullptr, B, sc.C, T, T, y, (long long)sc.C * T, T, 1, cx.st));
    return 0;
}

int fc_resblock_forward(fc_engine* e, const char* prefix, const float* x, int B, int T, float* y, void* workspace,
                        size_t workspace_bytes, void* stream) {
    return fc_resblock_forward_src(e, prefix, x, nullptr, nullptr, nullptr, B, T, y, workspace, workspace_bytes, stream);
}

int fc_lstm_forward(fc_engine* e, const char* prefix, const float* x, int B, int T, float* y, void* workspace,
                    size_t workspace_bytes, void* stream) {
    if (check_ready(e)) return 1;
    if (!prefix || !x || !y || B <= 0 || T <= 0) return fail("bad argument");
    auto it = e->lstm_by_prefix.find(prefix);
    if (it == e->lstm_by_prefix.end()) return fail(std::string("unknown lstm ") + prefix);
    Ctx cx = make_ctx(e, B, workspace, workspace_bytes, stream);
    Act in; in.raw = const_cast<float*>(x); in.C = it->second->H; in.T = T;
    Act o = run_lstm(e, cx, *it->second, in, T);
    if (cx.err) return 1;
    fc::Src s1;
    if (e->arch.lstm_skip) s1 = src_of(in);
    HIP_TRY(fc::launch_combine(src_of(o), s1, 0, 1.f, nullptr, B, o.C, T, T, y, (long long)o.C * T, T, 1, cx.st));
    return 0;
}

int fc_seq_forward(fc_engine* e, const char* prefix, const float* x, int B, int T, float* y, void* workspace,
                   size_t workspace_bytes, void* stream) {
    if (check_ready(e)) return 1;
    if (!prefix || !x || !y || B <= 0 || T <= 0) return fail("bad argument");
    auto it = e->tf_by_prefix.find(prefix);
    if (it == e->tf_by_prefix.end()) return fail(std::string("unknown transformer ") + prefix);
    Ctx cx = make_ctx(e, B, workspace, workspace_bytes, stream);
    Act in; in.raw = const_cast<float*>(x); in.C = it->second->C; in.T = T;
    Act o = run_transformer(e, cx, *it->second, in, T);
    if (cx.err) return 1;
    fc::Src s1;
    if (e->arch.lstm_skip) s1 = src_of(in);
    HIP_TRY(fc::launch_combine(src_of(o), s1, 0, 1.f, nullptr, B, o.C, T, T, y, (long long)o.C * T, T, 1, cx.st));
    return 0;
}

int fc_engine_status(fc_engine* e, unsigned* flags) {
    if (!e) return fail("null engine");
    unsigned f = 0;
    if (e->status_host) {
        if (e->status_host[FC_STATUS_LSTM_TIMEOUT]) f |= FC_STATUS_FLAG_LSTM_TIMEOUT;
        if (e->status_host[FC_STATUS_BAD_CODE]) f |= FC_STATUS_FLAG_BAD_CODE;
        if (e->status_host[FC_STATUS_BAD_LENGTH]) f |= FC_STATUS_FLAG_BAD_LENGTH;
    }
    if (flags) *flags = f;
    if (!e->finalized) return 0;
    return consume_status(e);
}

int fc_overlap_add(const float* const* frames, const int* lens, int n_frames, int B, int frame0_len, int stride, int out_len,
                   float* out, void* stream) {
    if (!frames || !lens || !out || n_frames <= 0 || B <= 0 || frame0_len <= 0 || stride <= 0 || out_len <= 0) return fail("bad argument");
    HIP_TRY(fc::launch_overlap_add(frames, lens, n_frames, B, frame0_len, stride, out_len, out, (hipStream_t)stream));
    return 0;
}

size_t fc_codec_json_bound(int n_q, int len) { return (size_t)(n_q > 0 ? n_q : 0) * ((size_t)(len > 0 ? len : 0) * 22 + 4) + 8; }

int fc_format_codec_json(const int64_t* codes, int n_q, int B, int T, int b, int len, char* out, size_t cap, size_t* written) {
    if (!codes || !out || !written || n_q <= 0 || B <= 0 || T <= 0 || b < 0 || b >= B || len < 0 || len > T) return fail("bad argument");
    if (cap < fc_codec_json_bound(n_q, len)) return fail("output buffer too small (fc_codec_json_bound)");
    char* p = out;
    *p++ = '['; *p++ = '[';
    for (int q = 0; q < n_q; ++q) {
        if (q) { *p++ = ','; *p++ = ' '; }
        *p++ = '[';
        const int64_t* row = codes + ((size_t)q * B + b) * T;
        for (int t = 0; t < len; ++t) {
            if (t) { *p++ = ','; *p++ = ' '; }
            long long v = row[t];
            if (v < 0) { *p++ = '-'; v = -v; }
            char tmp[24];
            int n = 0;
            do { tmp[n++] = (char)('0' + v % 10); v /= 10; } while (v);
            while (n) *p++ = tmp[--n];
        }
        *p++ = ']';
    }
    *p++ = ']'; *p++ = ']';
// ... 415 lines not shown
```

funcodec_amd/csrc/kernels.h:

```cpp
#pragma once
#include <hip/hip_runtime.h>
#include <stdint.h>
#include <stdio.h>
#include <stdlib.h>

#include <vector>

namespace fc {

inline int ab_knob(const char* name, int dflt) {
#ifdef FC_AB_KNOBS
    const char* v = getenv(name);
    return v ? atoi(v) : dflt;
#else
    if (getenv(name)) fprintf(stderr, "funcodec_amd: %s is set but ignored by this build (tuning knobs need FC_BUILD_DEFINES=FC_AB_KNOBS)\n", name);
    return dflt;
#endif
}

inline int deploy_switch(const char* name, int dflt) {
    const char* v = getenv(name);
    return v ? atoi(v) : dflt;
}

struct Src {
    const float* ptr = nullptr;
    const float* aff = nullptr;
    const float* div = nullptr;
    int used = 0;
    int ld = 0;
};

struct ConvLaunch {
    Src s0, s1;
    int elu = 0; float alpha = 1.f;
    const float* wt = nullptr;
    const float* bias = nullptr;
    const int* koff = nullptr;
    float* out = nullptr;
    long long out_sB = 0, out_sM = 0, out_sT = 1;
    int B = 0, Cin = 0, Tin = 0;
    int M = 0;
    int Tout = 0;
    int k = 1, stride = 1, padL = 0, padR = 0;
    int dil = 1;
    int pad_zero = 0;
    int up_r = 0, trimL = 0, Tfinal = 0;
    double* partials = nullptr;
    int BM = 128, BN = 128, CC = 2, nchunk = 1;
    int row = 0;
    int xq_Tp = 0;
    int Fo = 1;
    int affC = 0;
    long long in_sB0 = 0, in_sB1 = 0;
    long long out_sF = 0, part_sB0 = 0;
    int store_lo = 0, store_hi = 1 << 30;
    const float* w_plain = nullptr;
    float bias_host0 = 0.f;
};

int conv_nblk(const ConvLaunch& c);
bool conv_cout1_ok(const ConvLaunch& c);
bool conv_fewout_rows(const ConvLaunch& c);
void conv_fewout_name(const ConvLaunch& c, char* buf, size_t n);
size_t conv_lds_bytes(const ConvLaunch& c);
int conv_wbuf_floats(int k, int CC, int BM);
bool conv_quad(int CC);
size_t conv_pack_index(int k, int CC, int BM, int kk, int cl, int mm);
size_t conv_lds_bytes_for(int k, int stride, int dil, int CC, int BM, int BN, int Cin, int ntab, int row, int dma_rounds = -1);
bool conv_row_ok(int k, int stride, int dil, int CC, int BM, int BN, int Cin, bool dual);
bool conv_slab_fits(int k, int stride, int dil, int CC, int BN, int BM, bool dual);
int conv_wgs_per_cu(int BM);
std::vector<int> conv_koff_table(int k, int stride, int dil, int CC, int BN, int row);
hipError_t launch_conv(const ConvLaunch& c, hipStream_t st);
void conv_variant(const ConvLaunch& c, int* mode, int* nu, int* row);

struct ResHeadLaunch {
    Src s0, s1;
    const float *wsc = nullptr, *wb1 = nullptr;
    const float *bsc = nullptr, *bb1 = nullptr;
    float *out_sc = nullptr, *out_b1 = nullptr;
    double *part_sc = nullptr, *part_b1 = nullptr;
    int B = 0, C = 0, T = 0, k = 3, dil = 1, padL = 0, padR = 0;
    float alpha = 1.f;
};
bool reshead_ok(int C, int hid, int k_sc, int k_b1, int dil, int stride);
int reshead_ntiles(int T);
hipError_t launch_reshead(const ResHeadLaunch& c, hipStream_t st);

struct GConvLaunch {
    const float *src0 = nullptr, *aff0 = nullptr, *src1 = nullptr, *aff1 = nullptr;
    const float *w = nullptr, *bias = nullptr;
    float* out = nullptr;
    double* partials = nullptr;
    int B = 0, C = 0, M = 0, G = 1, Tin = 0, Tout = 0, Fo = 0, kf = 1, kt = 1, sf = 1, st = 1, padL = 0, padR = 0, elu = 0;
    float alpha = 1.f;
    long long in_sB = 0, in_sF = 0, out_sB = 0, out_sF = 0;
    const char *guard_lo = nullptr, *guard_hi = nullptr;
    int out_halo = 0;
};
bool gconv2d_ok(int cpg, int opg, int kf, int kt, int st);
bool gconv2d_fuses_halo(int kf, int kt, int st, int Fo, int halo);
int gconv2d_nblk(int Tout, int Fo, int G, int kf);
hipError_t launch_gconv2d(const GConvLaunch& c, hipStream_t st);
bool gconvtr2d_ok(int cpg, int opg, int tr);
int gconvtr2d_nblk(int Tin, int tr, int Fin, int fr);
hipError_t launch_gconvtr2d(const float* z, const float* w, const float* bias, float* out, double* partials, int B, int C, int cout, int Fin,
                            int Tin, int fr, int tr, int f_l, int Fout, int trimL, int Tout, long long out_sB, hipStream_t st,
                            int out_halo = 0 );
hipError_t launch_polyphase_in(const float* wav, const float* div, int B, int T, int hop, int n_fft, int Mp, float* xp, hipStream_t st);
hipError_t launch_stft_feats(const float* spec, int B, int F, int Tp, long long spec_sB, int halo, int C, float* feats, hipStream_t st);
hipError_t launch_feats_relayout(float* eng, float* ref, int B, int C, int F, int Tp, int halo, int to_ref, hipStream_t st);
hipError_t launch_halo_rows(float* buf, int B, int F, int halo, int C, int T, int zero, hipStream_t st);
hipError_t launch_halo_rows_short(float* buf, int B, int F, int halo, int pad, int C, int T, hipStream_t st);
hipError_t launch_combine2d(const float* s0, const float* aff0, int h0, const float* s1, const float* aff1, int h1, int elu, float alpha,
                            int B, int F, int C, int T, float* dst, int hd, hipStream_t st,
                            int halo_mode = 0 );
hipError_t launch_spec_from_dec(const float* dec, const float* aff, int B, int F, int Tp, int halo, int C, float* spec, hipStream_t st);
hipError_t launch_istft_finish(const float* ypoly, const float* win2, int B, int hop, int n_fft, int Mp, int Tp, const float* mul, int out_len,
                               float* wav, hipStream_t st);

hipError_t launch_gn_finalize(const double* partials, int nblk, double count, const float* gamma,
                              const float* beta, int C, float eps, int B, float* aff, hipStream_t st);

bool conv_xq_ok(int Cin, int CC, int k, int stride, int dil, int BM, int BN, int row);
size_t conv_xq_floats(int B, int Cin, int Tp, int BN, int stride, int k, int dil);
hipError_t launch_combine_xq(const Src& s0, const Src& s1, int elu, float alpha, int B, int C, int Tin, int padL, int padR, int pad_zero,
                             float* xq, hipStream_t st);

hipError_t launch_combine(const Src& s0, const Src& s1, int elu, float alpha, const float* mul,
                          int B, int C, int Tsrc, int Tcopy, float* out,
                          long long o_sB, long long o_sC, long long o_sT, hipStream_t st);

hipError_t launch_tanh_range(float* x, size_t n, float range, hipStream_t st);

hipError_t launch_volume(const float* wav , int B, int C, int T, float* scale, hipStream_t st,
                         const int* lens = nullptr);

hipError_t launch_transpose_btd(const float* in, int B, int T, int D, float* out, hipStream_t st);

hipError_t launch_rvq_encode(const float* x, int N, int D, int K, int nq, const float* cb, const float* cb_frag ,
                             const float* enorm,
                             int64_t* codes , float* quant ,
                             float* quant_bdt , float* subq ,
                             int Tf, hipStream_t st, const int* src0  = nullptr,
                             const int* nq_rows = nullptr);

__host__ __device__ inline int q0_source_frame(int t, int Tf) {
    const int half = Tf / 2;
    int j;
    if (Tf == 2 * half) j = t >> 1;
    else {
        const float up = (float)half / (float)Tf;
        j = (int)floorf((float)t * up);
        if (j > half - 1) j = half - 1;
    }
    const float down = (float)Tf / (float)half;
    int s = (int)floorf((float)j * down);
    if (s > Tf - 1) s = Tf - 1;
    return s;
}
hipError_t launch_q0_map(int* map , int B, int Tf, hipStream_t st);
hipError_t launch_rvq_decode(const int64_t* codes, int B, int Tf, int nq, int D, int K, const float* cb,
                             float* emb, float* emb_bdt, unsigned* status, hipStream_t st, const int* nq_rows = nullptr);

#define FC_STATUS_LSTM_TIMEOUT 0
#define FC_STATUS_BAD_CODE 1
#define FC_STATUS_BAD_LENGTH 2
#define FC_STATUS_WORDS 16

// ... 16 lines not shown
```

funcodec_amd/csrc/kernels.hip:

```cpp
#include "conv_kernel.h"

namespace fc {

#define FC_CONV_TILE(BM, BN, WM, WN) \
    extern template hipError_t launch_conv_tile<BM, BN, WM, WN>(const ConvLaunch&, const ConvArgs&, dim3, size_t, hipStream_t);
FC_CONV_TILE(128, 128, 2, 2)
FC_CONV_TILE(64, 256, 1, 4)
FC_CONV_TILE(32, 256, 1, 4)
FC_CONV_TILE(32, 128, 1, 4)
#undef FC_CONV_TILE
#define FC_CONV_TILE_Q(BM, BN, WM, WN) \
    extern template hipError_t launch_conv_tile_q<BM, BN, WM, WN>(const ConvLaunch&, const ConvArgs&, dim3, size_t, hipStream_t);
FC_CONV_TILE_Q(128, 128, 2, 2)
FC_CONV_TILE_Q(64, 256, 1, 4)
FC_CONV_TILE_Q(32, 256, 1, 4)
FC_CONV_TILE_Q(32, 128, 1, 4)
#undef FC_CONV_TILE_Q

bool conv_quad(int CC) {
    static const int quad_env = ab_knob("FC_QUAD", 1);
    return quad_env != 0 && CC >= 4 && CC % 4 == 0;
}
static int conv_nquads(int k, int CC) { return (((k * (CC / 4) + 1) / 2) + 1) & ~1; }
static int conv_koff_len(int k, int CC) { return conv_quad(CC) ? ((2 * conv_nquads(k, CC) + 3) & ~3) + 8 : (((k * CC / 2) + 3) & ~3) + 8; }
// ... 561 lines not shown
    float s1v = 0.f, s2v = 0.f;
    const int n0 = t0 + 4 * lane;
    const bool out_lane = wave_on && lane < C1_WOUT / 4;
#pragma unroll
    for (int m = 0; m < MO; ++m) {
        float o[4];
        const float bm = p.bias[m];
#pragma unroll
        for (int j = 0; j < 4; ++j) {
            o[j] = acc[m][j] + bm;
            if (out_lane && n0 + j < p.T) { s1v += o[j]; s2v = fmaf(o[j], o[j], s2v); }
        }
        if (FC_ABL(p.ablate, 2) || !out_lane) continue;
        float* orow = p.out + (size_t)breal * p.out_sB + (size_t)fo * p.out_sF + (size_t)m * p.out_sM + n0;
        if (n0 + 3 < p.T) *(f32x4u*)orow = (f32x4){o[0], o[1], o[2], o[3]};
        else
#pragma unroll
            for (int j = 0; j < 4; ++j) if (n0 + j < p.T) orow[j] = o[j];
    }
    fewout_partial(p, make_float2(s1v, s2v), red, breal, fo, tile);
}

bool conv_cout1_ok(const ConvLaunch& c) {
    return c.w_plain && c.M >= 1 && c.M <= 4 && c.store_lo <= 0 && c.store_hi >= c.Fo && c.stride == 1 && c.dil == 1 && !c.up_r && !c.pad_zero && !c.s0.div && c.out_sT == 1 && c.Tout == c.Tin &&
           (c.k == 7 || c.k == 3 || c.k == 5) && c.padL + c.padR == c.k - 1;
}

template <int K, int MO>
static hipError_t launch_fewout(const ConvLaunch& c, const Cout1Args& a, dim3 grid, hipStream_t st) {
    const dim3 block(256);
    if (conv_fewout_plain(c)) hipLaunchKernelGGL((conv_fewout_rows_plain_kernel<K, MO>), grid, block, 0, st, a);
    else if (conv_fewout_rows(c)) {
        if (c.s1.ptr) hipLaunchKernelGGL((conv_fewout_rows_kernel<K, true, MO>), grid, block, 0, st, a);
        else hipLaunchKernelGGL((conv_fewout_rows_kernel<K, false, MO>), grid, block, 0, st, a);
    } else {
        if (c.s1.ptr) hipLaunchKernelGGL((conv_cout1_kernel<K, true, MO>), grid, block, 0, st, a);
        else hipLaunchKernelGGL((conv_cout1_kernel<K, false, MO>), grid, block, 0, st, a);
    }
    return hipGetLastError();
}

static hipError_t launch_conv_cout1(const ConvLaunch& c, hipStream_t st) {
    Cout1Args a;
    a.src0 = c.s0.ptr; a.aff0 = c.s0.aff; a.src1 = c.s1.ptr; a.aff1 = c.s1.aff;
    a.w = c.w_plain; a.bias = c.bias; a.out = c.out; a.partials = c.partials;
    a.Cin = c.Cin; a.T = c.Tin; a.k = c.k; a.padL = c.padL;
    a.Fo = c.Fo > 1 ? c.Fo : 1; a.affC = c.affC > 0 ? c.affC : c.Cin;
    a.in_sB0 = c.in_sB0 ? c.in_sB0 : (long long)c.Cin * c.Tin; a.in_sB1 = c.in_sB1;
    a.out_sB = c.out_sB; a.out_sF = c.out_sF; a.out_sM = c.out_sM;
    const int tile_n = conv_fewout_tile(c);
    a.part_sB0 = c.part_sB0 ? c.part_sB0 : (long long)a.Fo * ceil_div(c.Tout, tile_n);
    static const int ablate_env = ab_knob("FC_ABLATE", 0);
    a.ablate = ablate_env;
    const int maxpad = c.padL > c.padR ? c.padL : c.padR;
    a.Leff = c.Tin > maxpad ? c.Tin : maxpad + 1;
    a.elu = c.elu; a.alpha = c.alpha;
    if (c.B > 65535) return hipErrorInvalidValue;
    const dim3 grid(ceil_div(c.Tout, tile_n), c.B);
    switch (10 * c.k + c.M) {
        case 31: return launch_fewout<3, 1>(c, a, grid, st);
        case 32: return launch_fewout<3, 2>(c, a, grid, st);
        case 33: return launch_fewout<3, 3>(c, a, grid, st);
        case 34: return launch_fewout<3, 4>(c, a, grid, st);
        case 51: return launch_fewout<5, 1>(c, a, grid, st);
        case 52: return launch_fewout<5, 2>(c, a, grid, st);
        case 53: return launch_fewout<5, 3>(c, a, grid, st);
        case 54: return launch_fewout<5, 4>(c, a, grid, st);
        case 71: return launch_fewout<7, 1>(c, a, grid, st);
        case 72: return launch_fewout<7, 2>(c, a, grid, st);
        case 73: return launch_fewout<7, 3>(c, a, grid, st);
        case 74: return launch_fewout<7, 4>(c, a, grid, st);
        default: return hipErrorInvalidValue;
    }
}

struct ResHeadArgs {
    const float *src0, *aff0, *src1, *aff1;
    const float *wsc, *wb1;
    const float *bsc, *bb1;
    float *out_sc, *out_b1;
    double *part_sc, *part_b1;
    int T, padL, padR, dil, Leff, ntiles;
    float alpha;
};
constexpr int RH_BN = 128, RH_XS = 144, RH_CH = 32;

__device__ __forceinline__ float wave_sum_f32(float v) {
    v += __builtin_bit_cast(float, __builtin_amdgcn_update_dpp(0, __builtin_bit_cast(int, v), 0xB1, 0xF, 0xF, false));
    v += __builtin_bit_cast(float, __builtin_amdgcn_update_dpp(0, __builtin_bit_cast(int, v), 0x4E, 0xF, 0xF, false));
    v += __builtin_bit_cast(float, __builtin_amdgcn_update_dpp(0, __builtin_bit_cast(int, v), 0x141, 0xF, 0xF, false));
    v += __builtin_bit_cast(float, __builtin_amdgcn_update_dpp(0, __builtin_bit_cast(int, v), 0x140, 0xF, 0xF, false));
    const float r0 = __builtin_bit_cast(float, __builtin_amdgcn_readlane(__builtin_bit_cast(int, v), 0));
    const float r1 = __builtin_bit_cast(float, __builtin_amdgcn_readlane(__builtin_bit_cast(int, v), 16));
    const float r2 = __builtin_bit_cast(float, __builtin_amdgcn_readlane(__builtin_bit_cast(int, v), 32));
    const float r3 = __builtin_bit_cast(float, __builtin_amdgcn_readlane(__builtin_bit_cast(int, v), 48));
    return ((r0 + r1) + r2) + r3;
}

template <int C, int K3, bool DUAL>
__global__ __launch_bounds__(256, C == 32 ? 3 : 2) void reshead_kernel(const ResHeadArgs p) {
    constexpr int HID = C / 2, NCH = C / RH_CH, MT = C / 32;
    constexpr bool B16 = HID == 16;
    extern __shared__ __attribute__((aligned(16))) float smem[];
    float* Wsc = smem;
    float* Wb1 = Wsc + C * C;
    float* Xa = Wb1 + K3 * C * HID;
    float* Xe = Xa + RH_CH * RH_XS;
    float* bias_s = Xe + RH_CH * RH_XS;
    float* red = bias_s + C + HID;

    const int tid = threadIdx.x, lane = tid & 63, wid = tid >> 6;
    const int hi = lane >> 5, l31 = lane & 31, g4 = lane >> 4, r16 = lane & 15;
    const int b = blockIdx.y;
    const int t_begin = (int)(((long long)p.ntiles * blockIdx.x) / gridDim.x);
    const int t_end = (int)(((long long)p.ntiles * (blockIdx.x + 1)) / gridDim.x);
    if (t_begin >= t_end) return;

    for (int i = tid * 4; i < C * C; i += 1024) *(f32x4*)(Wsc + i) = *(const f32x4*)(p.wsc + i);
    for (int i = tid * 4; i < K3 * C * HID; i += 1024) *(f32x4*)(Wb1 + i) = *(const f32x4*)(p.wb1 + i);
    for (int i = tid; i < C + HID; i += 256) bias_s[i] = i < C ? p.bsc[i] : p.bb1[i - C];

    const int halo = (K3 - 1) * p.dil;
    const int OFF = (4 - (p.padL & 3)) & 3;
    const int c4 = tid & 31, row0 = tid >> 5;
    const bool has_h = tid < RH_CH * halo;
    const int h_row = has_h ? tid / halo : 0, h_j = has_h ? tid - h_row * halo : 0;
    const int h_col = has_h ? (h_j < p.padL ? h_j - p.padL : RH_BN + (h_j - p.padL)) : 0;
    const size_t ubase = (size_t)b * C * p.T;
    const float* s0 = p.src0 + ubase;
    const float* s1 = DUAL ? p.src1 + ubase : s0;
    float2 A0[NCH][4], A1[DUAL ? NCH : 1][DUAL ? 4 : 1], Ah0[NCH], Ah1[DUAL ? NCH : 1];
#pragma unroll
    for (int ch = 0; ch < NCH; ++ch) {
#pragma unroll
        for (int r = 0; r < 4; ++r) {
            const int c = ch * RH_CH + row0 + 8 * r;
            A0[ch][r] = p.aff0 ? ((const float2*)p.aff0)[(size_t)b * C + c] : make_float2(1.f, 0.f);
            if (DUAL) A1[ch][r] = p.aff1 ? ((const float2*)p.aff1)[(size_t)b * C + c] : make_float2(1.f, 0.f);
        }
        const int c = ch * RH_CH + h_row;
        Ah0[ch] = p.aff0 ? ((const float2*)p.aff0)[(size_t)b * C + c] : make_float2(1.f, 0.f);
        if (DUAL) Ah1[ch] = p.aff1 ? ((const float2*)p.aff1)[(size_t)b * C + c] : make_float2(1.f, 0.f);
    }
    const int refl = 2 * (p.Leff - 1);
    auto resolve = [&](int g, bool& ok) __attribute__((always_inline)) {
        ok = g >= -p.padL && g < p.T + p.padR;
        int src = g < 0 ? -g : g;
        src = src >= p.Leff ? refl - src : src;
        ok = ok && src >= 0 && src < p.T;
        return ok ? src : 0;
    };

    f32x4 v0[2][4], v1[2][DUAL ? 4 : 1];
    float hv0[2] = {0.f, 0.f}, hv1[2] = {0.f, 0.f};
    unsigned vmask[2] = {0u, 0u};
    int ld_tile = 0, ld_chunk = 0, st_chunk = 0;
    auto load_item = [&](auto set_tag, auto fast_tag) __attribute__((always_inline)) {
        constexpr int S = decltype(set_tag)::value;
        constexpr bool FAST = decltype(fast_tag)::value;
        const int n0 = ld_tile * RH_BN, c0 = ld_chunk * RH_CH;
        if (++ld_chunk == NCH) { ld_chunk = 0; ++ld_tile; }
        if (FAST) {
#pragma unroll
            for (int r = 0; r < 4; ++r) {
                const size_t o = (size_t)(c0 + row0 + 8 * r) * p.T + n0 + 4 * c4;
                v0[S][r] = *(const f32x4u*)(s0 + o);
                if (DUAL) v1[S][r] = *(const f32x4u*)(s1 + o);
            }
            const size_t o = (size_t)(c0 + h_row) * p.T + n0 + h_col;
            hv0[S] = s0[o];
            if (DUAL) hv1[S] = s1[o];
        } else {
            unsigned vm = 0;
#pragma unroll
            for (int r = 0; r < 4; ++r) {
                const size_t ro = (size_t)(c0 + row0 + 8 * r) * p.T;
#pragma unroll
                for (int j = 0; j < 4; ++j) {
                    bool ok;
                    const int src = resolve(n0 + 4 * c4 + j, ok);
                    v0[S][r][j] = s0[ro + src];
                    if (DUAL) v1[S][r][j] = s1[ro + src];
                    vm |= (ok ? 1u : 0u) << (4 * r + j);
                }
            }
            bool ok;
            const int src = resolve(n0 + h_col, ok);
            const size_t o = (size_t)(c0 + h_row) * p.T + src;
            hv0[S] = s0[o];
            if (DUAL) hv1[S] = s1[o];
            vm |= (ok ? 1u : 0u) << 16;
            vmask[S] = vm;
        }
    };
    auto stage_item = [&](auto set_tag, auto fast_tag) __attribute__((always_inline)) {
        constexpr int S = decltype(set_tag)::value;
        constexpr bool FAST = decltype(fast_tag)::value;
        const int ch = st_chunk;
        if (++st_chunk == NCH) st_chunk = 0;
        const unsigned vm = FAST ? 0x1ffffu : vmask[S];
#pragma unroll
        for (int r = 0; r < 4; ++r) {
            const float2 A = NCH == 1 ? A0[0][r] : (ch ? A0[NCH - 1][r] : A0[0][r]);
            const float2 B1 = !DUAL ? make_float2(1.f, 0.f) : (NCH == 1 ? A1[0][DUAL ? r : 0] : (ch ? A1[DUAL ? NCH - 1 : 0][DUAL ? r : 0] : A1[0][DUAL ? r : 0]));
            f32x4 xa, xe;
#pragma unroll
            for (int j = 0; j < 4; ++j) {
                float v = fmaf(v0[S][r][j], A.x, A.y);
                if (DUAL) v = v + fmaf(v1[S][DUAL ? r : 0][j], B1.x, B1.y);
                float e = elu_f(v, p.alpha);
                if (!FAST) { const bool ok = (vm >> (4 * r + j)) & 1u; v = ok ? v : 0.f; e = ok ? e : 0.f; }
                xa[j] = v; xe[j] = e;
            }
            const int o = (row0 + 8 * r) * RH_XS + OFF + p.padL + 4 * c4;
            *(f32x4*)(Xa + o) = xa;
            *(f32x4*)(Xe + o) = xe;
        }
        {
            const float2 A = NCH == 1 ? Ah0[0] : (ch ? Ah0[NCH - 1] : Ah0[0]);
            const float2 B1 = !DUAL ? make_float2(1.f, 0.f) : (NCH == 1 ? Ah1[0] : (ch ? Ah1[DUAL ? NCH - 1 : 0] : Ah1[0]));
            float v = fmaf(hv0[S], A.x, A.y);
            if (DUAL) v = v + fmaf(hv1[S], B1.x, B1.y);
            float e = elu_f(v, p.alpha);
            if (!FAST) e = ((vm >> 16) & 1u) ? e : 0.f;
            if (has_h) Xe[h_row * RH_XS + OFF + p.padL + h_col] = e;
        }
    };

    f32x16 asc[MT];
    f32x16 ab32;
    f32x4 ab16[2];
    auto init_acc = [&]() __attribute__((always_inline)) {
#pragma unroll
        for (int mt = 0; mt < MT; ++mt)
#pragma unroll
            for (int r = 0; r < 16; ++r) asc[mt][r] = bias_s[mt * 32 + (r & 3) + 8 * (r >> 2) + 4 * hi];
        if (B16) {
#pragma unroll
            for (int j = 0; j < 2; ++j)
#pragma unroll
                for (int r = 0; r < 4; ++r) ab16[j][r] = bias_s[C + 4 * g4 + r];
        } else {
#pragma unroll
            for (int r = 0; r < 16; ++r) ab32[r] = bias_s[C + (r & 3) + 8 * (r >> 2) + 4 * hi];
        }
    };
    const int nl0 = wid * 32;
    using Set0 = std::integral_constant<int, 0>;
    using Set1 = std::integral_constant<int, 1>;
    __syncthreads();
    init_acc();

    auto item = [&](int f, int nitems, int& tile, int& chunk, auto set_tag, auto fast_tag) __attribute__((always_inline)) {
        constexpr bool FAST = decltype(fast_tag)::value;
        stage_item(set_tag, fast_tag);
        if (f + 2 < nitems) load_item(set_tag, fast_tag);
        __syncthreads();
        const int c0 = chunk * RH_CH;
        {
            const float* xb = Xa + hi * RH_XS + OFF + p.padL + nl0 + l31;
            const float* wa = Wsc + (c0 + hi) * C + l31;
#pragma unroll 2
            for (int ks = 0; ks < 16; ++ks) {
                const float bv = xb[2 * ks * RH_XS];
#pragma unroll
                for (int mt = 0; mt < MT; ++mt)
                    asc[mt] = __builtin_amdgcn_mfma_f32_32x32x2f32(wa[2 * ks * C + mt * 32], bv, asc[mt], 0, 0, 0);
            }
        }
        if (B16) {
#pragma unroll 1
            for (int kk = 0; kk < K3; ++kk) {
                const float* xb = Xe + g4 * RH_XS + OFF + nl0 + r16 + kk * p.dil;
                const float* wa = Wb1 + (kk * C + c0 + g4) * HID + r16;
#pragma unroll 4
                for (int q = 0; q < 8; ++q) {
                    const float av = wa[4 * q * HID];
                    ab16[0] = __builtin_amdgcn_mfma_f32_16x16x4f32(av, xb[4 * q * RH_XS], ab16[0], 0, 0, 0);
                    ab16[1] = __builtin_amdgcn_mfma_f32_16x16x4f32(av, xb[4 * q * RH_XS + 16], ab16[1], 0, 0, 0);
                }
            }
        } else {
#pragma unroll 1
            for (int kk = 0; kk < K3; ++kk) {
                const float* xb = Xe + hi * RH_XS + OFF + nl0 + l31 + kk * p.dil;
                const float* wa = Wb1 + (kk * C + c0 + hi) * HID + l31;
#pragma unroll 4
                for (int ks = 0; ks < 16; ++ks)
                    ab32 = __builtin_amdgcn_mfma_f32_32x32x2f32(wa[2 * ks * HID], xb[2 * ks * RH_XS], ab32, 0, 0, 0);
            }
        }
        const bool tile_done = chunk == NCH - 1;
        if (tile_done) {
            const int n0 = tile * RH_BN;
            float s1 = 0.f, s2 = 0.f, u1 = 0.f, u2 = 0.f;
            {
                const int col = n0 + nl0 + l31;
                const bool okc = FAST || col < p.T;
                float* o = p.out_sc + ubase + col + (size_t)(4 * hi) * p.T;
#pragma unroll
                for (int mt = 0; mt < MT; ++mt)
#pragma unroll
                    for (int r = 0; r < 16; ++r) {
                        const size_t mo = (size_t)(mt * 32 + (r & 3) + 8 * (r >> 2)) * p.T;
                        const float v = asc[mt][r];
                        if (FAST) { o[mo] = v; s1 += v; s2 = fmaf(v, v, s2); }
                        else if (okc) { o[mo] = v; s1 += v; s2 = fmaf(v, v, s2); }
                    }
            }
            float* ob = p.out_b1 + (size_t)b * HID * p.T;
            if (B16) {
                const int col = n0 + nl0 + r16;
                float* o = ob + col + (size_t)(4 * g4) * p.T;
#pragma unroll
                for (int j = 0; j < 2; ++j) {
#pragma unroll
                    for (int r = 0; r < 4; ++r) {
                        const float v = ab16[j][r];
                        const size_t mo = (size_t)r * p.T + 16 * j;
                        if (FAST) { o[mo] = v; u1 += v; u2 = fmaf(v, v, u2); }
                        else if (col + 16 * j < p.T) { o[mo] = v; u1 += v; u2 = fmaf(v, v, u2); }
                    }
                }
            } else {
                const int col = n0 + nl0 + l31;
                float* o = ob + col + (size_t)(4 * hi) * p.T;
#pragma unroll
                for (int r = 0; r < 16; ++r) {
                    const float v = ab32[r];
                    const size_t mo = (size_t)((r & 3) + 8 * (r >> 2)) * p.T;
                    if (FAST) { o[mo] = v; u1 += v; u2 = fmaf(v, v, u2); }
                    else if (col < p.T) { o[mo] = v; u1 += v; u2 = fmaf(v, v, u2); }
                }
            }
            if (p.part_sc) {
                const float w0 = wave_sum_f32(s1), w1 = wave_sum_f32(s2), w2 = wave_sum_f32(u1), w3 = wave_sum_f32(u2);
                if (lane == 0) *(f32x4*)(red + 4 * wid) = (f32x4){w0, w1, w2, w3};
            }
            init_acc();
        }
        __syncthreads();
        if (tile_done) {
            if (p.part_sc && tid < 4) {
                const int outp = tid >> 1, comp = tid & 1;
                double* dst = outp ? p.part_b1 : p.part_sc;
                const float* rr = red + outp * 2 + comp;
                dst[((size_t)b * p.ntiles + tile) * 2 + comp] = (((double)rr[0] + (double)rr[4]) + (double)rr[8]) + (double)rr[12];
            }
            ++tile; chunk = 0;
        } else {
            ++chunk;
        }
    };
    auto run = [&](int ta, int tb, auto fast_tag) __attribute__((always_inline)) {
        if (ta >= tb) return;
        const int nitems = (tb - ta) * NCH;
        ld_tile = ta; ld_chunk = 0; st_chunk = 0;
        int tile = ta, chunk = 0;
        load_item(Set0(), fast_tag);
        if (nitems > 1) load_item(Set1(), fast_tag);
        for (int f = 0; f < nitems; f += 2) {
            item(f, nitems, tile, chunk, Set0(), fast_tag);
            if (f + 1 < nitems) item(f + 1, nitems, tile, chunk, Set1(), fast_tag);
        }
    };
    int e0 = (p.padL + RH_BN - 1) / RH_BN;
    int e1 = p.T - p.padR - RH_BN >= 0 ? (p.T - p.padR - RH_BN) / RH_BN + 1 : 0;
    if (e1 < e0) e1 = e0;
    const int f0 = e0 < t_begin ? t_begin : (e0 > t_end ? t_end : e0);
    const int f1 = e1 < f0 ? f0 : (e1 > t_end ? t_end : e1);
    run(t_begin, f0, std::false_type());
    run(f0, f1, std::true_type());
    run(f1, t_end, std::false_type());
}

size_t reshead_lds_bytes(int C, int K3) {
    const int HID = C / 2;
    return (size_t)(C * C + K3 * C * HID + 2 * RH_CH * RH_XS + C + HID + 16) * sizeof(float);
}
int reshead_ntiles(int T) { return ceil_div(T, RH_BN); }
bool reshead_ok(int C, int hid, int k_sc, int k_b1, int dil, int stride) {
    return (C == 32 || C == 64) && hid * 2 == C && k_sc == 1 && stride == 1 && (k_b1 == 3 || k_b1 == 5 || k_b1 == 7) && (k_b1 - 1) * dil <= 8;
}

template <int C, int K3, bool DUAL>
static hipError_t launch_reshead_t(const ResHeadArgs& a, dim3 grid, size_t lds, hipStream_t st) {
    static std::atomic<unsigned long long> attr_done{0ull};
    auto kfn = reshead_kernel<C, K3, DUAL>;
    int dev = 0;
    (void)hipGetDevice(&dev);
    const unsigned long long bit = 1ull << (dev & 63);
    if (!(attr_done.load(std::memory_order_acquire) & bit)) {
        hipError_t ea = hipFuncSetAttribute((const void*)kfn, hipFuncAttributeMaxDynamicSharedMemorySize, 160 * 1024);
        if (ea != hipSuccess) return ea;
        attr_done.fetch_or(bit, std::memory_order_release);
    }
    hipLaunchKernelGGL(kfn, grid, dim3(256), lds, st, a);
    return hipGetLastError();
}

hipError_t launch_reshead(const ResHeadLaunch& c, hipStream_t st) {
    if (!reshead_ok(c.C, c.C / 2, 1, c.k, c.dil, 1)) return hipErrorInvalidValue;
    ResHeadArgs a;
    a.src0 = c.s0.ptr; a.aff0 = c.s0.aff; a.src1 = c.s1.ptr; a.aff1 = c.s1.aff;
    a.wsc = c.wsc; a.wb1 = c.wb1; a.bsc = c.bsc; a.bb1 = c.bb1;
    a.out_sc = c.out_sc; a.out_b1 = c.out_b1; a.part_sc = c.part_sc; a.part_b1 = c.part_b1;
    a.T = c.T; a.padL = c.padL; a.padR = c.padR; a.dil = c.dil;
    const int maxpad = c.padL > c.padR ? c.padL : c.padR;
    a.Leff = c.T > maxpad ? c.T : maxpad + 1;
    a.ntiles = reshead_ntiles(c.T);
    a.alpha = c.alpha;
    const size_t lds = reshead_lds_bytes(c.C, c.k);
    const int per_cu = (int)((160 * 1024) / lds) > 3 ? 3 : (int)((160 * 1024) / lds);
    static const int target_env = ab_knob("FC_RH_WGS", 0);
    const int target = target_env ? target_env : 256 * (per_cu < 1 ? 1 : per_cu);
    int G = target / c.B;
    if (G < 1) G = 1;
    if (G > a.ntiles) G = a.ntiles;
    dim3 grid(G, c.B);
    const bool dual = c.s1.ptr != nullptr;
#define FC_RH(CC, KK)                                                                              \
    if (c.C == CC && c.k == KK)                                                                    \
        return dual ? launch_reshead_t<CC, KK, true>(a, grid, lds, st) : launch_reshead_t<CC, KK, false>(a, grid, lds, st);
    FC_RH(32, 3) FC_RH(64, 3) FC_RH(32, 5) FC_RH(64, 5) FC_RH(32, 7) FC_RH(64, 7)
#undef FC_RH
    return hipErrorInvalidValue;
}

__global__ __launch_bounds__(256) void gn_finalize_kernel(const double* __restrict__ partials, int nblk, double count,
                                                          const float* __restrict__ gamma, const float* __restrict__ beta,
                                                          int C, float eps, float* __restrict__ aff) {
    __shared__ double sh[2][256];
    const int b = blockIdx.x, tid = threadIdx.x;
    double s1 = 0.0, s2 = 0.0;
    for (int i = tid; i < nblk; i += 256) {
        s1 += partials[((size_t)b * nblk + i) * 2];
        s2 += partials[((size_t)b * nblk + i) * 2 + 1];
    }
    sh[0][tid] = s1; sh[1][tid] = s2;
    __syncthreads();
    for (int o = 128; o >= 1; o >>= 1) {
        if (tid < o) { sh[0][tid] += sh[0][tid + o]; sh[1][tid] += sh[1][tid + o]; }
        __syncthreads();
    }
    const double mean = sh[0][0] / count;
    double var = sh[1][0] / count - mean * mean;
    if (var < 0.0) var = 0.0;
    const float rstd = (float)(1.0 / sqrt(var + (double)eps));
    const float meanf = (float)mean;
    for (int c = tid; c < C; c += 256) {
        const float a = rstd * gamma[c];
        const float s = fmaf(-a, meanf, beta[c]);
        ((float2*)aff)[(size_t)b * C + c] = make_float2(a, s);
    }
}

hipError_t launch_gn_finalize(const double* partials, int nblk, double count, const float* gamma, const float* beta,
                              int C, float eps, int B, float* aff, hipStream_t st) {
    hipLaunchKernelGGL(gn_finalize_kernel, dim3(B), dim3(256), 0, st, partials, nblk, count, gamma, beta, C, eps, aff);
    return hipGetLastError();
}

__global__ __launch_bounds__(256) void combine_kernel(Src s0, Src s1, int elu, float alpha, const float* __restrict__ mul,
                                                      int C, int Tsrc, int Tcopy, float* __restrict__ out,
                                                      long long o_sB, long long o_sC, long long o_sT) {
    const int b = blockIdx.z, c = blockIdx.y;
    const size_t row = (size_t)b * C + c;
    float2 a0 = make_float2(1.f, 0.f), a1 = make_float2(1.f, 0.f);
    if (s0.aff) a0 = ((const float2*)s0.aff)[row];
    if (s1.ptr && s1.aff) a1 = ((const float2*)s1.aff)[row];
    const float m = mul ? mul[b] : 1.f;
    if (o_sT == 1 && !s0.div) {
        float* orow = out + (size_t)b * o_sB + (size_t)c * o_sC;
        const float* r0 = s0.ptr + row * Tsrc;
        const float* r1 = s1.ptr ? s1.ptr + row * Tsrc : r0;
        const int T4 = Tcopy >> 2;
        for (int q = blockIdx.x * 256 + threadIdx.x; q < T4; q += gridDim.x * 256) {
            const f32x4 x0 = *(const f32x4u*)(r0 + 4 * q);
            const f32x4 x1 = s1.ptr ? (f32x4)(*(const f32x4u*)(r1 + 4 * q)) : x0;
            f32x4 y;
#pragma unroll
            for (int j = 0; j < 4; ++j) {
                float v = x0[j];
                if (s0.aff) v = fmaf(v, a0.x, a0.y);
                if (s1.ptr) {
                    float w = x1[j];
                    if (s1.aff) w = fmaf(w, a1.x, a1.y);
                    v = v + w;
                }
                if (elu) v = elu_f(v, alpha);
                if (mul) v = v * m;
                y[j] = v;
            }
            *(f32x4u*)(orow + 4 * q) = y;
        }
        for (int t = 4 * T4 + blockIdx.x * 256 + threadIdx.x; t < Tcopy; t += gridDim.x * 256) {
            float v = r0[t];
            if (s0.aff) v = fmaf(v, a0.x, a0.y);
            if (s1.ptr) {
                float w = r1[t];
                if (s1.aff) w = fmaf(w, a1.x, a1.y);
                v = v + w;
            }
            if (elu) v = elu_f(v, alpha);
            if (mul) v = v * m;
            orow[t] = v;
        }
        return;
    }
// ... 1063 lines not shown
```

funcodec_amd/engine.py:

```python
from __future__ import annotations

import contextlib
import ctypes as C
import logging
from typing import Dict, Optional

import numpy as np
import torch

from . import _lib
from .config import SEQ_FF, SEQ_HEADS, ArchSpec


class EngineError(RuntimeError):
    pass


def _ptr(t: Optional[torch.Tensor]):
    return None if t is None else C.c_void_p(t.data_ptr())


def _on_device(fn):
    import functools

# ... 454 lines not shown
    def layer2d_forward(self, prefix: str, x0: torch.Tensor, aff0: Optional[torch.Tensor] = None, x1: Optional[torch.Tensor] = None,
                        aff1: Optional[torch.Tensor] = None, apply_elu: bool = False, out_halo: int = 0) -> torch.Tensor:
        x0 = self._dev(x0, torch.float32)
        if x0.dim() != 4:
            raise EngineError(f"layer2d_forward: x0 must be [B,C,F,T], got {tuple(x0.shape)}")
        B, Cin, Fq, T = x0.shape
        dims = (C.c_int64 * 5)()
        self._check(self.lib.fc_layer2d_out_shape(self._h, prefix.encode(), B, Fq, T, int(out_halo), dims))
        if Cin != int(dims[4]):
            raise EngineError(f"layer {prefix}: expected input [B, {int(dims[4])}, F, T], got {tuple(x0.shape)}")
        srcs = [(x0, aff0)] + ([(x1, aff1)] if x1 is not None else [])
        if x1 is None and aff1 is not None:
            raise EngineError("layer2d_forward: aff1 without x1")
        conv = []
        for x, a in srcs:
            x = self._dev(x, torch.float32)
            if tuple(x.shape) != (B, Cin, Fq, T):
                raise EngineError(f"layer2d_forward: every source must be [B,C,F,T] = {(B, Cin, Fq, T)}, got {tuple(x.shape)}")
            if a is not None:
                a = self._dev(a, torch.float32)
                if tuple(a.shape) != (B, Cin, 2):
                    raise EngineError(f"layer2d_forward: an affine must be [B,C,2] = {(B, Cin, 2)}, got {tuple(a.shape)}")
            conv.append((x, a))
        y = torch.empty((B, int(dims[0]), int(dims[1]), int(dims[2])), dtype=torch.float32, device=self.device)
        need = int(dims[3])
        ws = self._scratch(need)
        (s0, a0), (s1, a1) = conv[0], (conv[1] if len(conv) > 1 else (None, None))
        self._check(self.lib.fc_layer2d_forward(self._h, prefix.encode(), _ptr(s0), _ptr(a0), _ptr(s1), _ptr(a1), B, Fq, T, int(apply_elu),
                                                int(out_halo), _ptr(y), _ptr(ws), ws.numel(), self._stream()))
        return y

    @_on_device
    def freq_synthesis(self, dec: torch.Tensor, aff: Optional[torch.Tensor] = None, scale: Optional[torch.Tensor] = None,
                       out_len: Optional[int] = None, want_spec: bool = False):
        dec = self._dev(dec, torch.float32)
        if dec.dim() != 4:
            raise EngineError(f"freq_synthesis: dec must be [B,C,F,Tp], got {tuple(dec.shape)}")
        B, Cc, Fq, Tp = dec.shape
        if out_len is None:
            out_len = self.arch.stft_hop * (Tp - 1)
        need = C.c_size_t()
        self._check(self.lib.fc_freq_synthesis_size(self._h, B, Cc, Fq, Tp, int(out_len), C.byref(need)))
        if aff is not None:
            aff = self._dev(aff, torch.float32)
            if tuple(aff.shape) != (B, Cc, 2):
                raise EngineError(f"freq_synthesis: the affine must be [B,C,2] = {(B, Cc, 2)}, got {tuple(aff.shape)}")
        if scale is not None:
            scale = self._dev(scale.reshape(-1), torch.float32)
            if scale.numel() != B:
                raise EngineError(f"freq_synthesis: scale must hold one value per utterance ({B}), got {scale.numel()}")
        wav = torch.empty((B, int(out_len)), dtype=torch.float32, device=self.device)
        spec = torch.empty((B, 2 * Fq, Tp), dtype=torch.float32, device=self.device) if want_spec else None
        ws = self._scratch(need.value)
        self._check(self.lib.fc_freq_synthesis(self._h, _ptr(dec), _ptr(aff), _ptr(scale), B, Cc, Fq, Tp, int(out_len), _ptr(wav), _ptr(spec),
                                               _ptr(ws), ws.numel(), self._stream()))
        return (wav, spec) if want_spec else wav

    def freq_halo(self) -> int:
        dims = (C.c_int64 * 5)()
        for k in self.expected_tensors():
            if k.endswith(".conv.bias") and k.startswith("encoder.model.0."):
                self._check(self.lib.fc_layer2d_out_shape(self._h, k[:-len(".conv.bias")].encode(), 1, 1, 1, -1, dims))
                return int(dims[0])
        raise EngineError("freq_halo: not an STFT-domain codec")

    @_on_device
    def resblock_forward(self, prefix: str, x: torch.Tensor, *, aff0: Optional[torch.Tensor] = None, x1: Optional[torch.Tensor] = None,
                         aff1: Optional[torch.Tensor] = None) -> torch.Tensor:
        x = self._dev(x, torch.float32)
        B, Cc, T = x.shape
        x1, aff0, aff1 = self._sources(f"block {prefix}", x.shape, aff0, x1, aff1)
        y = torch.empty_like(x)
        need = B * Cc * (T + 64) * 4 * 6 + (4 << 20)
        ws = self._scratch(need)
        if aff0 is None and x1 is None:
            rc = self.lib.fc_resblock_forward(self._h, prefix.encode(), _ptr(x), B, T, _ptr(y), _ptr(ws), ws.numel(), self._stream())
        else:
            rc = self.lib.fc_resblock_forward_src(self._h, prefix.encode(), _ptr(x), _ptr(aff0), _ptr(x1), _ptr(aff1), B, T, _ptr(y), _ptr(ws),
                                                  ws.numel(), self._stream())
        self._check(rc)
        return y

    @_on_device
    def lstm_forward(self, prefix: str, x: torch.Tensor) -> torch.Tensor:
        x = self._dev(x, torch.float32)
        B, H, T = x.shape
        want = self.expected_tensors().get(prefix + ".weight_hh_l0")
        if want is None or want[1] != H:
            raise EngineError(f"lstm {prefix!r}: expected input [B, {want[1] if want else '?'}, T], got {tuple(x.shape)}")
        y = torch.empty_like(x)
        need = (T * B * 4 * H + 3 * B * H + B * H * T + (2 * T + 1) * 16 * ((B + 15) // 16) * H) * 4 * self.arch.lstm_layers + (1 << 20)
        ws = self._scratch(need)
        self._check(self.lib.fc_lstm_forward(self._h, prefix.encode(), _ptr(x), B, T, _ptr(y), _ptr(ws), ws.numel(), self._stream()))
        return y

    @_on_device
    def seq_forward(self, prefix: str, x: torch.Tensor) -> torch.Tensor:
        x = self._dev(x, torch.float32)
        B, Cc, T = x.shape
        want = self.expected_tensors().get(prefix + ".after_norm.weight")
        if want is None or want[0] != Cc:
            raise EngineError(f"transformer {prefix!r}: expected input [B, {want[0] if want else '?'}, T], got {tuple(x.shape)}")
        y = torch.empty_like(x)
        need = 4 * B * T * (8 * Cc + SEQ_FF) + (1 << 20)
        ws = self._scratch(need)
        self._check(self.lib.fc_seq_forward(self._h, prefix.encode(), _ptr(x), B, T, _ptr(y), _ptr(ws), ws.numel(), self._stream()))
        return y

    @_on_device
    def stream_seq_forward(self, session, x: torch.Tensor, decoder: bool = False) -> torch.Tensor:
        x = self._dev(x, torch.float32)
        B, Cc, T = x.shape
        if B != session.batch or Cc != self.arch.bottleneck_channels:
            raise EngineError(f"stream_seq_forward: x must be [{session.batch},{self.arch.bottleneck_channels},T], got {tuple(x.shape)}")
        y = torch.empty_like(x)
        need = 4 * B * T * (8 * Cc + SEQ_FF) + 4 * B * 256 * (Cc + 2 * SEQ_HEADS) + (1 << 20)
        ws = self._scratch(need)
        self._check(self.lib.fc_seqstream_forward(session._h, int(decoder), _ptr(x), T, _ptr(y), _ptr(ws), ws.numel(), self._stream()))
        return y
```

include/funcodec_amd.h:

```cpp
#ifndef FUNCODEC_AMD_H
#define FUNCODEC_AMD_H

#include <stddef.h>
#include <stdint.h>

#ifdef __cplusplus
extern "C" {
#endif

#define FC_MAX_RATIOS 8
#define FC_ABI_VERSION 7

typedef struct fc_engine fc_engine;

typedef struct fc_arch {
    int32_t abi_version;
    int32_t sample_rate;
    int32_t audio_normalize;
    int32_t n_filters;
    int32_t dimension;
    int32_t n_ratios;
    int32_t ratios[FC_MAX_RATIOS];
    int32_t kernel_size;
    int32_t last_kernel_size;
// ... 71 lines not shown

int fc_overlap_add(const float* const* frames, const int* lens, int n_frames, int B, int frame0_len, int stride,
                   int out_len, float* out, void* stream);

typedef struct fc_stream fc_stream;
size_t fc_stream_state_bytes(const fc_engine* e, int B);
int  fc_stream_create(fc_engine* e, int B, int max_chunk_samples, int n_q, void* state , size_t state_bytes, fc_stream** out);
void fc_stream_destroy(fc_stream* s);
int  fc_stream_min_first(const fc_stream* s, int decode);
size_t fc_stream_workspace_bytes(const fc_stream* s);
int  fc_stream_reset(fc_stream* s, const float* scale, void* stream);
int  fc_stream_encode(fc_stream* s, const float* wav, int Tc, int final, int64_t* codes, float* quantized, float* enc_out, int* n_frames,
                      void* workspace, size_t workspace_bytes, void* stream);
int  fc_stream_decode_codes(fc_stream* s, const int64_t* codes, int Tfc, int use_scale, float* wav, float* emb_out,
                            void* workspace, size_t workspace_bytes, void* stream);
int  fc_stream_decode_emb(fc_stream* s, const float* emb, int Tfc, int use_scale, float* wav,
                          void* workspace, size_t workspace_bytes, void* stream);

int  fc_stream_lstm_forward(fc_stream* s, int decoder, const float* x, int T, float* y, void* workspace, size_t workspace_bytes, void* stream);

size_t fc_seqstream_state_bytes(const fc_engine* e, int B, int max_frames);
int  fc_seqstream_create(fc_engine* e, int B, int max_chunk_samples, int n_q, int max_frames, void* state , size_t state_bytes,
                         fc_stream** out);
int  fc_seqstream_forward(fc_stream* s, int decoder, const float* x, int T, float* y, void* workspace, size_t workspace_bytes, void* stream);

#define FC_SLOT_START 1
#define FC_SLOT_FINAL 2
typedef struct fc_slots fc_slots;
size_t fc_slots_state_bytes(const fc_engine* e, int S);
int  fc_slots_create(fc_engine* e, int S, int max_chunk_samples, int n_q, void* state , size_t state_bytes, fc_slots** out);
void fc_slots_destroy(fc_slots* s);
int  fc_slots_min_first(const fc_slots* s, int decode);
size_t fc_slots_workspace_bytes(const fc_slots* s);
int  fc_slots_encode(fc_slots* s, const float* wav, int Tc, const int32_t* samples, const int32_t* flags, const float* scale, int64_t* codes,
                     float* quantized, float* enc_out, void* workspace, size_t workspace_bytes, void* stream);
int  fc_slots_decode_codes(fc_slots* s, const int64_t* codes, int Tfc, const int32_t* frames, const int32_t* flags, int use_scale, float* wav,
                           float* emb_out, void* workspace, size_t workspace_bytes, void* stream);
int  fc_slots_decode_emb(fc_slots* s, const float* emb, int Tfc, const int32_t* frames, const int32_t* flags, int use_scale, float* wav,
                         void* workspace, size_t workspace_bytes, void* stream);
int  fc_slots_lstm_forward(fc_slots* s, int decoder, const float* x, int T, const int32_t* steps, const int32_t* start, float* y,
                           void* workspace, size_t workspace_bytes, void* stream);

size_t fc_seqslots_state_bytes(const fc_engine* e, int S, int max_frames);
int  fc_seqslots_create(fc_engine* e, int S, int max_chunk_samples, int n_q, int max_frames, void* state , size_t state_bytes,
                        fc_slots** out);
int  fc_seqslots_forward(fc_slots* s, int decoder, const float* x, int T, const int32_t* frames, const int32_t* start, float* y,
                         void* workspace, size_t workspace_bytes, void* stream);

int  fc_graphstream_set(fc_stream* s, int on);
int  fc_graphstream_enabled(const fc_stream* s);
int  fc_graphstream_counts(const fc_stream* s, int64_t counts[4]);
int  fc_graphslots_set(fc_slots* s, int on);
int  fc_graphslots_enabled(const fc_slots* s);
int  fc_graphslots_counts(const fc_slots* s, int64_t counts[4]);

#define FC_STATUS_FLAG_LSTM_TIMEOUT 1u
#define FC_STATUS_FLAG_BAD_CODE 2u
#define FC_STATUS_FLAG_BAD_LENGTH 4u
int fc_engine_status(fc_engine* e, unsigned* flags);

int fc_rvq_encode(fc_engine* e, const float* x, int N, int n_q, int64_t* codes, float* quantized,
                  void* workspace, size_t workspace_bytes, void* stream);

int fc_q0_source_frames(int Tf, int32_t* frames );

int fc_layer_forward(fc_engine* e, const char* prefix, const float* x, int B, int T, int apply_elu,
                     float* y, void* workspace, size_t workspace_bytes, void* stream);
int fc_layer_forward_src(fc_engine* e, const char* prefix, const float* x0, const float* aff0, const float* div0, const float* x1,
                         const float* aff1, int B, int T, int apply_elu, float* y, void* workspace, size_t workspace_bytes, void* stream);
int fc_layer_out_len(const fc_engine* e, const char* prefix, int T);

int fc_layer2d_forward(fc_engine* e, const char* prefix, const float* x0, const float* aff0, const float* x1, const float* aff1,
                       int B, int F, int T, int apply_elu, int out_halo, float* y, void* workspace, size_t workspace_bytes, void* stream);
int fc_layer2d_out_shape(const fc_engine* e, const char* prefix, int B, int F, int T, int out_halo, int64_t* dims );

int fc_freq_synthesis(fc_engine* e, const float* dec, const float* aff, const float* scale, int B, int C, int F, int Tp, int out_len,
                      float* wav, float* spec, void* workspace, size_t workspace_bytes, void* stream);
int fc_freq_synthesis_size(const fc_engine* e, int B, int C, int F, int Tp, int out_len, size_t* workspace_bytes);

int fc_resblock_forward(fc_engine* e, const char* prefix, const float* x, int B, int T,
                        float* y, void* workspace, size_t workspace_bytes, void* stream);
int fc_resblock_forward_src(fc_engine* e, const char* prefix, const float* x0, const float* aff0, const float* x1, const float* aff1,
                            int B, int T, float* y, void* workspace, size_t workspace_bytes, void* stream);

int fc_lstm_forward(fc_engine* e, const char* prefix, const float* x, int B, int T,
                    float* y, void* workspace, size_t workspace_bytes, void* stream);

int fc_seq_forward(fc_engine* e, const char* prefix, const float* x, int B, int T,
                   float* y, void* workspace, size_t workspace_bytes, void* stream);

typedef struct fc_work {
    double total_flops, total_bytes;
    double conv_flops, conv_bytes;
    double lstm_flops, rvq_flops;
    int32_t conv_launches, total_launches;
} fc_work;
int fc_engine_work(const fc_engine* e, int B, int T, int n_q, fc_work* out);

typedef struct fc_prof {
    char    kernel[64];
    double  total_ms;
    double  flops, bytes;
    int32_t launches;
    int32_t reserved;
} fc_prof;
#define FC_PROF_CLASSES 48
int fc_engine_profile(fc_engine* e, int enable);
int fc_engine_profile_read(fc_engine* e, fc_prof* out );

int fc_debug_timeline(unsigned long long* dst );

int fc_debug_conv_layout(int k, int stride, int dil, int CC, int BM, int BN, int row, int* info , int* pack_index, size_t pack_cap,
                         int* koff, size_t koff_cap);

int fc_debug_freq_features(void* dev_buf, size_t cap_bytes, int mode);

size_t fc_codec_json_bound(int n_q, int len);
int fc_format_codec_json(const int64_t* codes, int n_q, int B, int T, int b, int len, char* out, size_t cap, size_t* written);
int fc_write_wav_pcm16(const char* path, const float* wav, int n, int sample_rate, int rescale);

typedef struct fc_laura fc_laura;

typedef struct fc_laura_stack {
    int32_t idim, d_model, heads, ff, layers;
    int32_t act;
    int32_t embed_relu;
    int32_t norm_style;
} fc_laura_stack;

typedef struct fc_laura_arch {
    int32_t abi_version;
    int32_t input_size;
    int32_t vocab_size;
    int32_t codebook_size;
    int32_t codebook_dim;
    int32_t num_quantizers;
    int32_t predict_nq;
    int32_t pos_emb_split;
    int32_t bidirectional_inputs;
    int32_t max_positions;
    fc_laura_stack text_encoder, codec_lm, codec_encoder;
} fc_laura_arch;

int  fc_laura_create(const fc_laura_arch* arch, int device, fc_laura** out);
void fc_laura_destroy(fc_laura* e);
int  fc_laura_num_weights(const fc_laura* e);
int  fc_laura_weight_info(const fc_laura* e, int i, const char** name, int64_t* dims);
int  fc_laura_set_weight(fc_laura* e, const char* name, const float* host, const int64_t* dims, int ndim);
int  fc_laura_finalize(fc_laura* e);
size_t fc_laura_workspace_bytes(const fc_laura* e, int B, int L, int Cmax, int max_length);

int fc_laura_encode(fc_laura* e, const float* text_emb, const int64_t* text_ids, const int32_t* text_lens, int B, int L,
                    float* text_outs, void* workspace, size_t workspace_bytes, void* stream);

int fc_laura_lm_logprobs(fc_laura* e, const float* text_outs, const int32_t* text_lens, int B, int L, const int64_t* codec,
                         const int32_t* codec_lens, int Cmax, float* logp, int Tseq, void* workspace, size_t workspace_bytes, void* stream);

int fc_laura_decode_codec(fc_laura* e, const float* text_outs, const int32_t* text_lens, int B, int L, const int64_t* continual,
                          const int32_t* cont_lens, int Cmax, int max_length, int sampling_mode, int sampling_k, float sampling_p,
                          uint64_t seed, const int64_t* forced, int64_t* tokens, int32_t* out_lens, float* step_logp,
                          void* workspace, size_t workspace_bytes, void* stream);

int fc_laura_codec_emb(fc_laura* e, const float* text_outs, const int32_t* text_lens, int B, int L, const int64_t* codec, int nq_cols,
                       const int32_t* codec_lens, int Cmax, float* emb, void* workspace, size_t workspace_bytes, void* stream);

int fc_laura_linear(fc_laura* e, const char* name, const float* x, int B, int T, int step_form, float* y,
// ... 53 lines not shown
```

Before: 10710 audio-s/s.

## Fold encoder first conv into fused res-block head kernel, recomputing it from waveform

The encoder's first 1->32 channel k=7 conv is no longer materialized. A small stats-only kernel computes its GroupNorm statistics, and the first res-block head kernel recomputes the conv per tile from the raw waveform staged in LDS. This removes writing and re-reading a 32-channel full-rate activation, at the cost of extra recompute and more LDS in the head kernel. A debug entry point compares the folded and unfolded paths.

```diff
diff --git a/funcodec_amd/_lib.py b/funcodec_amd/_lib.py
--- a/funcodec_amd/_lib.py
+++ b/funcodec_amd/_lib.py
@@ -91,6 +91,7 @@
     "fc_seq_forward": (C.c_int, [_P, C.c_char_p, _P, C.c_int, C.c_int, _P, _P, C.c_size_t, _P]),
     "fc_resblock_forward": (C.c_int, [_P, C.c_char_p, _P, C.c_int, C.c_int, _P, _P, C.c_size_t, _P]),
     "fc_resblock_forward_src": (C.c_int, [_P, C.c_char_p, _P, _P, _P, _P, C.c_int, C.c_int, _P, _P, C.c_size_t, _P]),
+    "fc_debug_encoder_head": (C.c_int, [_P, _P, _P, C.c_int, C.c_int, C.c_int, _P, _P, _P, _P, _P, C.c_size_t, _P]),
     "fc_engine_work": (C.c_int, [_P, C.c_int, C.c_int, C.c_int, C.POINTER(FcWork)]),
     "fc_engine_profile": (C.c_int, [_P, C.c_int]),
     "fc_engine_profile_read": (C.c_int, [_P, C.POINTER(FcProf)]),
diff --git a/funcodec_amd/csrc/engine.hip b/funcodec_amd/csrc/engine.hip
--- a/funcodec_amd/csrc/engine.hip
+++ b/funcodec_amd/csrc/engine.hip
@@ -146,6 +146,8 @@
     std::vector<int32_t> row_nq;
     int* row_nq_dev = nullptr;
     size_t row_nq_cap = 0;
+    bool head_fold = true;
+    float* head_w = nullptr;
     bool lstm_persist_ok = true;
     int persist_checked_B = -1; bool persist_checked_val = false;
     bool profiling = false;
@@ -842,6 +844,20 @@
     if (upload(e, e->host[R.shortcut.prefix + ".conv.bias"].data, &R.bsc)) return 1;
     if (upload(e, e->host[R.block1.prefix + ".conv.bias"].data, &R.bb1)) return 1;
     return 0;
+}
+
+int pack_head_fold(fc_engine* e) {
+    const ConvLayer& L = e->enc_first;
+    if (e->enc_stages.empty() || e->enc_stages[0].res.empty() || !e->enc_stages[0].res[0].fused_head) return 0;
+    if (L.cin != 1 || L.cout != 32 || L.k != 7 || L.stride != 1 || L.dil != 1 || !L.has_norm || L.transposed) return 0;
+    const auto& W = e->host[L.prefix + ".conv.weight"].data;
+    const auto& Bv = e->host[L.prefix + ".conv.bias"].data;
+    std::vector<float> h((size_t)32 * 8);
+    for (int m = 0; m < 32; ++m) {
+        for (int kk = 0; kk < 7; ++kk) h[(size_t)m * 8 + kk] = W[(size_t)m * 7 + kk];
+        h[(size_t)m * 8 + 7] = Bv[m];
+    }
+    return upload(e, h, &e->head_w);
 }
 
 
@@ -1274,7 +1290,24 @@
     return tb.C ? run_transformer(e, cx, tb, in, T) : run_lstm(e, cx, lb, in, T);
 }
 
-void run_reshead(fc_engine* e, Ctx& cx, const fc_engine::ResBlock& R, fc::Src a0, fc::Src a1, int T, Act* sc, Act* b1) {
+Act run_head_stats(fc_engine* e, Ctx& cx, const fc::Src& wav, int T) {
+    const ConvLayer& L = e->enc_first;
+    const ConvGeom g = conv_geom(L, T);
+    Act out;
+    out.C = L.cout; out.T = T; out.normed = true;
+    const int nblk = fc::head_stats_ntiles(T);
+    double* partials = cx.alloc<double>((size_t)cx.B * nblk * 2);
+    out.aff = cx.alloc<float>((size_t)cx.B * L.cout * 2);
+    const double fl = 2.0 * cx.B * (double)L.M * L.cin * L.gk * T, by = 4.0 * cx.B * (double)T;
+    cx.conv_flops += fl; cx.conv_bytes += by;
+    cx.conv_launch("first conv statistics", L.prefix.c_str(), [] { return "head_stats_kernel"; }, fl, by,
+                   [&] { return fc::launch_head_stats(wav.ptr, wav.div, e->head_w, partials, cx.B, T, g.padL, g.padR, cx.st); });
+    conv_finish(e, cx, L, partials, nblk, (double)L.cout * T, out.aff);
+    return out;
+}
+
+void run_reshead(fc_engine* e, Ctx& cx, const fc_engine::ResBlock& R, fc::Src a0, fc::Src a1, int T, Act* sc, Act* b1, const fc::Src* wav = nullptr,
+                 double** parts_out = nullptr) {
     const int C = R.shortcut.cin, hid = R.block1.cout;
     const ConvGeom g = conv_geom(R.block1, T);
     sc->C = C; sc->T = T; b1->C = hid; b1->T = T;
@@ -1285,6 +1318,11 @@
     c.out_sc = sc->raw; c.out_b1 = b1->raw;
     c.B = cx.B; c.C = C; c.T = T; c.k = R.block1.k; c.dil = R.block1.dil; c.padL = g.padL; c.padR = g.padR;
     c.alpha = e->arch.elu_alpha;
+    if (wav) {
+        const ConvGeom g1 = conv_geom(e->enc_first, T);
+        c.s0.ptr = wav->ptr;
+        c.head_w = e->head_w; c.head_div = wav->div; c.head_k = e->enc_first.k; c.head_padL = g1.padL; c.head_padR = g1.padR;
+    }
     const int nblk = fc::reshead_ntiles(T);
     if (R.shortcut.has_norm) {
         c.part_sc = cx.alloc<double>((size_t)cx.B * nblk * 2);
@@ -1293,16 +1331,17 @@
         b1->aff = cx.alloc<float>((size_t)cx.B * hid * 2); b1->normed = true;
     }
     const double fl = 2.0 * cx.B * (double)T * ((double)C * C + (double)hid * C * R.block1.k);
-    const double by = 4.0 * cx.B * (double)T * ((double)C * (a1.used ? 2 : 1) + C + hid);
+    const double by = 4.0 * cx.B * (double)T * ((wav ? 1.0 : (double)C * (a1.used ? 2 : 1)) + C + hid);
     cx.conv_flops += fl; cx.conv_bytes += by;
     auto cls = [&] {
         char nm[64];
-        snprintf(nm, sizeof(nm), "reshead_kernel<%d, %d, %s>", C, R.block1.k, a1.used ? "true" : "false");
+        snprintf(nm, sizeof(nm), "reshead_kernel<%d, %d, %s%s>", C, R.block1.k, a1.used ? "true" : "false", wav ? ", true" : "");
         return std::string(nm);
     };
     cx.conv_launch("fused res-block head", R.shortcut.prefix.c_str(), cls, fl, by, [&] { return fc::launch_reshead(c, cx.st); });
     conv_finish(e, cx, R.shortcut, c.part_sc, nblk, (double)C * T, sc->aff);
     conv_finish(e, cx, R.block1, c.part_b1, nblk, (double)hid * T, b1->aff);
+    if (parts_out) { parts_out[0] = c.part_sc; parts_out[1] = c.part_b1; }
 }
 
 struct Pass {
@@ -1378,11 +1417,12 @@
     if (e->arch.lstm_skip) *a1 = src_of(x);
 }
 
-void run_resblocks(fc_engine* e, Ctx& cx, const Pass& p, const fc_engine::Stage& S, fc::Src a0, fc::Src a1, int T, Act* sc, Act* b3) {
+void run_resblocks(fc_engine* e, Ctx& cx, const Pass& p, const fc_engine::Stage& S, fc::Src a0, fc::Src a1, int T, Act* sc, Act* b3,
+                   const fc::Src* wav = nullptr) {
     for (const auto& R : S.res) {
         Act b1;
         if (p.kind == Pass::Offline && R.fused_head && !a0.div) {
-            run_reshead(e, cx, R, a0, a1, T, sc, &b1);
+            run_reshead(e, cx, R, a0, a1, T, sc, &b1, &R == &S.res[0] ? wav : nullptr);
         } else {
             *sc = walk_conv(e, cx, p, Role::Shortcut, R.shortcut, a0, a1, 0, T);
             b1 = walk_conv(e, cx, p, Role::Block1, R.block1, a0, a1, 1, T);
@@ -1394,10 +1434,16 @@
 
 Act run_encoder(fc_engine* e, Ctx& cx, const Pass& p, fc::Src wav, int T) {
     cx.dec_side = false; cx.rate = 1; cx.no_xq = p.kind == Pass::Ragged;
-    Act x = walk_conv(e, cx, p, Role::First, e->enc_first, wav, fc::Src(), 0, T);
+    const ConvGeom g1 = conv_geom(e->enc_first, T);
+    const bool fold = e->head_fold && e->head_w && p.kind == Pass::Offline && !wav.aff && !e->enc_stages.empty() && !e->enc_stages[0].res.empty() &&
+                      e->enc_stages[0].res[0].fused_head && g1.Tout == T &&
+                      fc::reshead_head_ok(e->enc_first.cout, e->enc_first.k, g1.padL, g1.padR, conv_geom(e->enc_stages[0].res[0].block1, T).padL,
+                                          conv_geom(e->enc_stages[0].res[0].block1, T).padR);
+    Act x = fold ? run_head_stats(e, cx, wav, T)
+                 : walk_conv(e, cx, p, Role::First, e->enc_first, wav, fc::Src(), 0, T);
     for (auto& S : e->enc_stages) {
         Act sc, b3;
-        run_resblocks(e, cx, p, S, src_of(x), fc::Src(), x.T, &sc, &b3);
+        run_resblocks(e, cx, p, S, src_of(x), fc::Src(), x.T, &sc, &b3, fold && &S == &e->enc_stages[0] ? &wav : nullptr);
         x = walk_conv(e, cx, p, Role::Resample, S.resample, src_of(sc), src_of(b3), 1, sc.T);
         cx.rate *= S.resample.stride;
     }
@@ -2405,6 +2451,7 @@
     fc_engine* e = new fc_engine();
     e->arch = *arch;
     e->device = device;
+    e->head_fold = fc::deploy_switch("FC_HEAD_FOLD", 1) != 0;
     build_plan(e);
     for (const auto& kv : e->by_prefix)
         if (kv.second->unsupported) {
@@ -2526,7 +2573,7 @@
         int err = 0;
         for_each_conv(e, [&](const ConvVisit& v) { if (!err && v.role == Role::Shortcut) err = pack_reshead(e, *v.block); });
         for_each_conv(e, [&](const ConvVisit& v) { if (!err) err = pack_conv(e, v.L); });
-        if (err) return 1;
+        if (err || pack_head_fold(e)) return 1;
     }
     if (pack_lstm(e, e->enc_lstm)) return 1;
     if (pack_lstm(e, e->dec_lstm)) return 1;
@@ -2981,6 +3028,29 @@
     run_resblocks(e, cx, Pass(), one, hook_src(x0, aff0, nullptr), hook_src(x1, aff1, nullptr), T, &sc, &b3);
     if (cx.err) return 1;
     HIP_TRY(fc::launch_combine(src_of(sc), src_of(b3), 0, 1.f, nullptr, B, sc.C, T, T, y, (long long)sc.C * T, T, 1, cx.st));
+    return 0;
+}
+
+int fc_debug_encoder_head(fc_engine* e, const float* wav, const float* div, int B, int T, int fold, float* sc_raw, float* b1_raw, double* part_sc,
+                          double* part_b1, void* workspace, size_t workspace_bytes, void* stream) {
+    if (!e || !wav || !sc_raw || !b1_raw || B <= 0 || T <= 0) return fail("bad argument");
+    if (check_ready(e)) return 1;
+    if (e->arch.model_type != 0 || e->enc_stages.empty() || e->enc_stages[0].res.empty() || !e->enc_stages[0].res[0].fused_head)
+        return fail("fc_debug_encoder_head: the encoder's first block has no fused head");
+    if (fold && !e->head_w) return fail("fc_debug_encoder_head: this net's first conv cannot be folded into the head");
+    const fc_engine::ResBlock& R = e->enc_stages[0].res[0];
+    Ctx cx = make_ctx(e, B, workspace, workspace_bytes, stream);
+    const fc::Src w = hook_src(wav, nullptr, div);
+    Act x = fold ? run_head_stats(e, cx, w, T) : run_conv(e, cx, e->enc_first, w, fc::Src(), 0, T);
+    Act sc, b1;
+    double* parts[2] = {nullptr, nullptr};
+    run_reshead(e, cx, R, src_of(x), fc::Src(), T, &sc, &b1, fold ? &w : nullptr, parts);
+    if (cx.err) return 1;
+    const size_t nt = (size_t)fc::reshead_ntiles(T);
+    HIP_TRY(hipMemcpyAsync(sc_raw, sc.raw, (size_t)B * sc.C * T * sizeof(float), hipMemcpyDeviceToDevice, cx.st));
+    HIP_TRY(hipMemcpyAsync(b1_raw, b1.raw, (size_t)B * b1.C * T * sizeof(float), hipMemcpyDeviceToDevice, cx.st));
+    if (part_sc && parts[0]) HIP_TRY(hipMemcpyAsync(part_sc, parts[0], (size_t)B * nt * 2 * sizeof(double), hipMemcpyDeviceToDevice, cx.st));
+    if (part_b1 && parts[1]) HIP_TRY(hipMemcpyAsync(part_b1, parts[1], (size_t)B * nt * 2 * sizeof(double), hipMemcpyDeviceToDevice, cx.st));
     return 0;
 }
 
diff --git a/funcodec_amd/csrc/kernels.h b/funcodec_amd/csrc/kernels.h
--- a/funcodec_amd/csrc/kernels.h
+++ b/funcodec_amd/csrc/kernels.h
@@ -83,9 +83,14 @@
     double *part_sc = nullptr, *part_b1 = nullptr;
     int B = 0, C = 0, T = 0, k = 3, dil = 1, padL = 0, padR = 0;
     float alpha = 1.f;
+    const float *head_w = nullptr, *head_div = nullptr;
+    int head_k = 0, head_padL = 0, head_padR = 0;
 };
 bool reshead_ok(int C, int hid, int k_sc, int k_b1, int dil, int stride);
+bool reshead_head_ok(int C, int k_first, int padL_first, int padR_first, int padL, int padR);
 int reshead_ntiles(int T);
+int head_stats_ntiles(int T);
+hipError_t launch_head_stats(const float* wav, const float* div, const float* w, double* partials, int B, int T, int padL, int padR, hipStream_t st);
 hipError_t launch_reshead(const ResHeadLaunch& c, hipStream_t st);
 
 struct GConvLaunch {
diff --git a/funcodec_amd/csrc/kernels.hip b/funcodec_amd/csrc/kernels.hip
--- a/funcodec_amd/csrc/kernels.hip
+++ b/funcodec_amd/csrc/kernels.hip
@@ -667,8 +667,11 @@
     double *part_sc, *part_b1;
     int T, padL, padR, dil, Leff, ntiles;
     float alpha;
+    const float *head_w, *head_div;
+    int head_padL, head_padR, head_Leff;
 };
 constexpr int RH_BN = 128, RH_XS = 144, RH_CH = 32;
+constexpr int RH_K1 = 7, RH_WS = 160;
 
 __device__ __forceinline__ float wave_sum_f32(float v) {
     v += __builtin_bit_cast(float, __builtin_amdgcn_update_dpp(0, __builtin_bit_cast(int, v), 0xB1, 0xF, 0xF, false));
@@ -682,8 +685,9 @@
     return ((r0 + r1) + r2) + r3;
 }
 
-template <int C, int K3, bool DUAL>
+template <int C, int K3, bool DUAL, bool HEAD = false>
 __global__ __launch_bounds__(256, C == 32 ? 3 : 2) void reshead_kernel(const ResHeadArgs p) {
+    static_assert(!HEAD || (C == 32 && !DUAL), "the HEAD form: 32 channels, one source");
     constexpr int HID = C / 2, NCH = C / RH_CH, MT = C / 32;
     constexpr bool B16 = HID == 16;
     extern __shared__ __attribute__((aligned(16))) float smem[];
@@ -693,6 +697,8 @@
     float* Xe = Xa + RH_CH * RH_XS;
     float* bias_s = Xe + RH_CH * RH_XS;
     float* red = bias_s + C + HID;
+    float* Wv = red + 16;
+    float* H1 = Wv + 2 * RH_WS;
 
     const int tid = threadIdx.x, lane = tid & 63, wid = tid >> 6;
     const int hi = lane >> 5, l31 = lane & 31, g4 = lane >> 4, r16 = lane & 15;
@@ -704,6 +710,7 @@
     for (int i = tid * 4; i < C * C; i += 1024) *(f32x4*)(Wsc + i) = *(const f32x4*)(p.wsc + i);
     for (int i = tid * 4; i < K3 * C * HID; i += 1024) *(f32x4*)(Wb1 + i) = *(const f32x4*)(p.wb1 + i);
     for (int i = tid; i < C + HID; i += 256) bias_s[i] = i < C ? p.bsc[i] : p.bb1[i - C];
+    if (HEAD) H1[tid] = p.head_w[tid];
 
     const int halo = (K3 - 1) * p.dil;
     const int OFF = (4 - (p.padL & 3)) & 3;
@@ -712,8 +719,11 @@
     const int h_row = has_h ? tid / halo : 0, h_j = has_h ? tid - h_row * halo : 0;
     const int h_col = has_h ? (h_j < p.padL ? h_j - p.padL : RH_BN + (h_j - p.padL)) : 0;
     const size_t ubase = (size_t)b * C * p.T;
-    const float* s0 = p.src0 + ubase;
+    const float* s0 = HEAD ? p.src0 + (size_t)b * p.T : p.src0 + ubase;
     const float* s1 = DUAL ? p.src1 + ubase : s0;
+    const int hpl = HEAD ? p.head_padL : 0, hpr = HEAD ? p.head_padR : 0;
+    const int WSP = RH_BN + halo + RH_K1 - 1;
+    const float hdivv = (HEAD && p.head_div) ? p.head_div[b] : 1.f;
     float2 A0[NCH][4], A1[DUAL ? NCH : 1][DUAL ? 4 : 1], Ah0[NCH], Ah1[DUAL ? NCH : 1];
 #pragma unroll
     for (int ch = 0; ch < NCH; ++ch) {
@@ -740,6 +750,35 @@
     float hv0[2] = {0.f, 0.f}, hv1[2] = {0.f, 0.f};
     unsigned vmask[2] = {0u, 0u};
     int ld_tile = 0, ld_chunk = 0, st_chunk = 0;
+    float wv2[2] = {0.f, 0.f};
+    bool wv_ok2[2] = {true, true};
+    int st_tile = 0, wcur = 0;
+    auto load_wave = [&](auto set_tag, auto fast_tag) __attribute__((always_inline)) {
+        constexpr int S = decltype(set_tag)::value;
+        constexpr bool FAST = decltype(fast_tag)::value;
+        float& wv = wv2[S];
+        bool& wv_ok = wv_ok2[S];
+        const int q = ld_tile * RH_BN - p.padL - hpl + (tid < WSP ? tid : WSP - 1);
+        ++ld_tile;
+        if (FAST) {
+            wv = s0[q];
+        } else {
+            bool ok = q >= -hpl && q < p.T + hpr;
+            int src = q < 0 ? -q : q;
+            src = src >= p.head_Leff ? 2 * (p.head_Leff - 1) - src : src;
+            ok = ok && src >= 0 && src < p.T;
+            wv = s0[ok ? src : 0];
+            wv_ok = ok;
+        }
+    };
+    auto wave_to_lds = [&](int buf, auto set_tag, auto fast_tag) __attribute__((always_inline)) {
+        constexpr int S = decltype(set_tag)::value;
+        constexpr bool FAST = decltype(fast_tag)::value;
+        float v = wv2[S];
+        if (p.head_div) { v = v / hdivv; v = fmaf(v, 1.f, 0.f); }
+        if (!FAST) v = wv_ok2[S] ? v : 0.f;
+        if (tid < WSP) Wv[buf * RH_WS + OFF + tid] = v;
+    };
     auto load_item = [&](auto set_tag, auto fast_tag) __attribute__((always_inline)) {
         constexpr int S = decltype(set_tag)::value;
         constexpr bool FAST = decltype(fast_tag)::value;
@@ -783,7 +822,52 @@
         constexpr bool FAST = decltype(fast_tag)::value;
         const int ch = st_chunk;
         if (++st_chunk == NCH) st_chunk = 0;
-        const unsigned vm = FAST ? 0x1ffffu : vmask[S];
+        unsigned vm = FAST ? 0x1ffffu : vmask[S];
+        f32x4 hx[HEAD ? 4 : 1];
+        float hxh = 0.f;
+        if constexpr (HEAD) {
+            const float* wb = Wv + wcur * RH_WS + OFF;
+            const int n0s = st_tile * RH_BN;
+            ++st_tile;
+            auto span_of = [&](int lcol, bool& ok) __attribute__((always_inline)) {
+                const int i = resolve(n0s + lcol, ok) - n0s + p.padL;
+                return i < 0 ? 0 : (i > WSP - RH_K1 ? WSP - RH_K1 : i);
+            };
+            auto conv1 = [&](const float (&x)[RH_K1], int row) __attribute__((always_inline)) {
+                const f32x4 ta = *(const f32x4*)(H1 + row * 8), tb = *(const f32x4*)(H1 + row * 8 + 4);
+                float a = tb[3];
+                a = fmaf(ta[0], x[0], a); a = fmaf(ta[1], x[1], a); a = fmaf(ta[2], x[2], a); a = fmaf(ta[3], x[3], a);
+                a = fmaf(tb[0], x[4], a); a = fmaf(tb[1], x[5], a); a = fmaf(tb[2], x[6], a);
+                return a + 0.f;
+            };
+            int hidx = h_col + p.padL;
+            if (FAST) {
+                const f32x4* wq = (const f32x4*)(wb + p.padL + 4 * c4);
+                const f32x4 q0 = wq[0], q1 = wq[1], q2 = wq[2];
+                const float xw[12] = {q0[0], q0[1], q0[2], q0[3], q1[0], q1[1], q1[2], q1[3], q2[0], q2[1], q2[2], q2[3]};
+#pragma unroll
+                for (int r = 0; r < 4; ++r)
+#pragma unroll
+                    for (int j = 0; j < 4; ++j) {
+                        const float xj[RH_K1] = {xw[j], xw[j + 1], xw[j + 2], xw[j + 3], xw[j + 4], xw[j + 5], xw[j + 6]};
+                        hx[r][j] = conv1(xj, row0 + 8 * r);
+                    }
+            } else {
+                bool ok;
+                hidx = span_of(h_col, ok);
+                vm = ok ? 0x10000u : 0u;
+#pragma unroll
+                for (int j = 0; j < 4; ++j) {
+                    const int i = span_of(4 * c4 + j, ok);
+                    vm |= (ok ? 0x1111u : 0u) << j;
+                    const float xj[RH_K1] = {wb[i], wb[i + 1], wb[i + 2], wb[i + 3], wb[i + 4], wb[i + 5], wb[i + 6]};
+#pragma unroll
+                    for (int r = 0; r < 4; ++r) hx[r][j] = conv1(xj, row0 + 8 * r);
+                }
+            }
+            const float xh[RH_K1] = {wb[hidx], wb[hidx + 1], wb[hidx + 2], wb[hidx + 3], wb[hidx + 4], wb[hidx + 5], wb[hidx + 6]};
+            hxh = conv1(xh, h_row);
+        }
 #pragma unroll
         for (int r = 0; r < 4; ++r) {
             const float2 A = NCH == 1 ? A0[0][r] : (ch ? A0[NCH - 1][r] : A0[0][r]);
@@ -791,7 +875,7 @@
             f32x4 xa, xe;
 #pragma unroll
             for (int j = 0; j < 4; ++j) {
-                float v = fmaf(v0[S][r][j], A.x, A.y);
+                float v = fmaf(HEAD ? hx[HEAD ? r : 0][j] : v0[S][r][j], A.x, A.y);
                 if (DUAL) v = v + fmaf(v1[S][DUAL ? r : 0][j], B1.x, B1.y);
                 float e = elu_f(v, p.alpha);
                 if (!FAST) { const bool ok = (vm >> (4 * r + j)) & 1u; v = ok ? v : 0.f; e = ok ? e : 0.f; }
@@ -804,7 +888,7 @@
         {
             const float2 A = NCH == 1 ? Ah0[0] : (ch ? Ah0[NCH - 1] : Ah0[0]);
             const float2 B1 = !DUAL ? make_float2(1.f, 0.f) : (NCH == 1 ? Ah1[0] : (ch ? Ah1[DUAL ? NCH - 1 : 0] : Ah1[0]));
-            float v = fmaf(hv0[S], A.x, A.y);
+            float v = fmaf(HEAD ? hxh : hv0[S], A.x, A.y);
             if (DUAL) v = v + fmaf(hv1[S], B1.x, B1.y);
             float e = elu_f(v, p.alpha);
             if (!FAST) e = ((vm >> 16) & 1u) ? e : 0.f;
@@ -839,6 +923,9 @@
     auto item = [&](int f, int nitems, int& tile, int& chunk, auto set_tag, auto fast_tag) __attribute__((always_inline)) {
         constexpr bool FAST = decltype(fast_tag)::value;
         stage_item(set_tag, fast_tag);
+        if constexpr (HEAD) {
+            if (f + 2 < nitems) load_wave(set_tag, fast_tag);
+        } else
         if (f + 2 < nitems) load_item(set_tag, fast_tag);
         __syncthreads();
         const int c0 = chunk * RH_CH;
@@ -875,6 +962,11 @@
                     ab32 = __builtin_amdgcn_mfma_f32_32x32x2f32(wa[2 * ks * HID], xb[2 * ks * RH_XS], ab32, 0, 0, 0);
             }
         }
+        if constexpr (HEAD) {
+            using Other = std::integral_constant<int, 1 - decltype(set_tag)::value>;
+            if (f + 1 < nitems) wave_to_lds(wcur ^ 1, Other(), fast_tag);
+            wcur ^= 1;
+        }
         const bool tile_done = chunk == NCH - 1;
         if (tile_done) {
             const int n0 = tile * RH_BN;
@@ -942,15 +1034,24 @@
         const int nitems = (tb - ta) * NCH;
         ld_tile = ta; ld_chunk = 0; st_chunk = 0;
         int tile = ta, chunk = 0;
+        if constexpr (HEAD) {
+            st_tile = ta; wcur = 0;
+            load_wave(Set0(), fast_tag);
+            wave_to_lds(0, Set0(), fast_tag);
+            if (nitems > 1) load_wave(Set1(), fast_tag);
+            __syncthreads();
+        } else {
         load_item(Set0(), fast_tag);
         if (nitems > 1) load_item(Set1(), fast_tag);
+        }
         for (int f = 0; f < nitems; f += 2) {
             item(f, nitems, tile, chunk, Set0(), fast_tag);
             if (f + 1 < nitems) item(f + 1, nitems, tile, chunk, Set1(), fast_tag);
         }
     };
-    int e0 = (p.padL + RH_BN - 1) / RH_BN;
-    int e1 = p.T - p.padR - RH_BN >= 0 ? (p.T - p.padR - RH_BN) / RH_BN + 1 : 0;
+    const int extL = p.padL + hpl, extR = p.padR + hpr;
+    int e0 = (extL + RH_BN - 1) / RH_BN;
+    int e1 = p.T - extR - RH_BN >= 0 ? (p.T - extR - RH_BN) / RH_BN + 1 : 0;
     if (e1 < e0) e1 = e0;
     const int f0 = e0 < t_begin ? t_begin : (e0 > t_end ? t_end : e0);
     const int f1 = e1 < f0 ? f0 : (e1 > t_end ? t_end : e1);
@@ -959,19 +1060,22 @@
     run(f1, t_end, std::false_type());
 }
 
-size_t reshead_lds_bytes(int C, int K3) {
+size_t reshead_lds_bytes(int C, int K3, bool head = false) {
     const int HID = C / 2;
-    return (size_t)(C * C + K3 * C * HID + 2 * RH_CH * RH_XS + C + HID + 16) * sizeof(float);
+    return (size_t)(C * C + K3 * C * HID + 2 * RH_CH * RH_XS + C + HID + 16 + (head ? 2 * RH_WS + C * 8 : 0)) * sizeof(float);
 }
 int reshead_ntiles(int T) { return ceil_div(T, RH_BN); }
 bool reshead_ok(int C, int hid, int k_sc, int k_b1, int dil, int stride) {
     return (C == 32 || C == 64) && hid * 2 == C && k_sc == 1 && stride == 1 && (k_b1 == 3 || k_b1 == 5 || k_b1 == 7) && (k_b1 - 1) * dil <= 8;
 }
-
-template <int C, int K3, bool DUAL>
+bool reshead_head_ok(int C, int k_first, int padL_first, int padR_first, int padL, int padR) {
+    return C == 32 && k_first == RH_K1 && padL_first >= 0 && padR_first >= 0 && padL_first + padR_first == RH_K1 - 1 && padR <= padL;
+}
+
+template <int C, int K3, bool DUAL, bool HEAD = false>
 static hipError_t launch_reshead_t(const ResHeadArgs& a, dim3 grid, size_t lds, hipStream_t st) {
     static std::atomic<unsigned long long> attr_done{0ull};
-    auto kfn = reshead_kernel<C, K3, DUAL>;
+    auto kfn = reshead_kernel<C, K3, DUAL, HEAD>;
     int dev = 0;
     (void)hipGetDevice(&dev);
     const unsigned long long bit = 1ull << (dev & 63);
@@ -995,7 +1099,12 @@
     a.Leff = c.T > maxpad ? c.T : maxpad + 1;
     a.ntiles = reshead_ntiles(c.T);
     a.alpha = c.alpha;
-    const size_t lds = reshead_lds_bytes(c.C, c.k);
+    const bool head = c.head_w != nullptr;
+    if (head && (c.s1.ptr || !reshead_head_ok(c.C, c.head_k, c.head_padL, c.head_padR, c.padL, c.padR))) return hipErrorInvalidValue;
+    a.head_w = c.head_w; a.head_div = c.head_div; a.head_padL = c.head_padL; a.head_padR = c.head_padR;
+    const int maxpad1 = c.head_padL > c.head_padR ? c.head_padL : c.head_padR;
+    a.head_Leff = c.T > maxpad1 ? c.T : maxpad1 + 1;
+    const size_t lds = reshead_lds_bytes(c.C, c.k, head);
     const int per_cu = (int)((160 * 1024) / lds) > 3 ? 3 : (int)((160 * 1024) / lds);
     static const int target_env = ab_knob("FC_RH_WGS", 0);
     const int target = target_env ? target_env : 256 * (per_cu < 1 ? 1 : per_cu);
@@ -1004,12 +1113,100 @@
     if (G > a.ntiles) G = a.ntiles;
     dim3 grid(G, c.B);
     const bool dual = c.s1.ptr != nullptr;
+    if (head) {
+        if (c.k == 3) return launch_reshead_t<32, 3, false, true>(a, grid, lds, st);
+        if (c.k == 5) return launch_reshead_t<32, 5, false, true>(a, grid, lds, st);
+        if (c.k == 7) return launch_reshead_t<32, 7, false, true>(a, grid, lds, st);
+        return hipErrorInvalidValue;
+    }
 #define FC_RH(CC, KK)                                                                              \
     if (c.C == CC && c.k == KK)                                                                    \
         return dual ? launch_reshead_t<CC, KK, true>(a, grid, lds, st) : launch_reshead_t<CC, KK, false>(a, grid, lds, st);
     FC_RH(32, 3) FC_RH(64, 3) FC_RH(32, 5) FC_RH(64, 5) FC_RH(32, 7) FC_RH(64, 7)
 #undef FC_RH
     return hipErrorInvalidValue;
+}
+
+struct HeadStatsArgs {
+    const float *wav, *div, *w;
+    double* partials;
+    int T, padL, padR, Leff, ntiles;
+};
+constexpr int HS_BN = 256;
+__global__ __launch_bounds__(256) void head_stats_kernel(const HeadStatsArgs p) {
+    __shared__ __attribute__((aligned(16))) float xs[HS_BN + 8];
+    __shared__ __attribute__((aligned(16))) float ws[256];
+    __shared__ float2 red[256];
+    const int tid = threadIdx.x, lane = tid & 63, wid = tid >> 6, hi = lane >> 5, l31 = lane & 31;
+    const int b = blockIdx.y;
+    const float* w0 = p.wav + (size_t)b * p.T;
+    const float divv = p.div ? p.div[b] : 1.f;
+    ws[tid] = p.w[tid];
+    for (int tile = blockIdx.x; tile < p.ntiles; tile += gridDim.x) {
+        const int n0 = tile * HS_BN;
+        for (int i = tid; i < HS_BN + RH_K1 - 1; i += 256) {
+            const int q = n0 - p.padL + i;
+            bool ok = q >= -p.padL && q < p.T + p.padR;
+            int src = q < 0 ? -q : q;
+            src = src >= p.Leff ? 2 * (p.Leff - 1) - src : src;
+            ok = ok && src >= 0 && src < p.T;
+            float v = w0[ok ? src : 0];
+            if (p.div) { v = v / divv; v = fmaf(v, 1.f, 0.f); }
+            xs[i] = ok ? v : 0.f;
+        }
+        __syncthreads();
+        float x[2][RH_K1];
+        bool okc[2];
+#pragma unroll
+        for (int j = 0; j < 2; ++j) {
+            const int c = wid * 64 + j * 32 + l31;
+            okc[j] = n0 + c < p.T;
+#pragma unroll
+            for (int kk = 0; kk < RH_K1; ++kk) x[j][kk] = xs[c + kk];
+        }
+        float s1 = 0.f, s2 = 0.f;
+#pragma unroll
+        for (int r = 0; r < 16; ++r) {
+            const int m = (r & 3) + 8 * (r >> 2) + 4 * hi;
+            const f32x4 ta = *(const f32x4*)(ws + m * 8), tb = *(const f32x4*)(ws + m * 8 + 4);
+#pragma unroll
+            for (int j = 0; j < 2; ++j) {
+                float a = tb[3];
+                a = fmaf(ta[0], x[j][0], a); a = fmaf(ta[1], x[j][1], a); a = fmaf(ta[2], x[j][2], a); a = fmaf(ta[3], x[j][3], a);
+                a = fmaf(tb[0], x[j][4], a); a = fmaf(tb[1], x[j][5], a); a = fmaf(tb[2], x[j][6], a);
+                const float v = a + 0.f;
+                if (okc[j]) { s1 += v; s2 = fmaf(v, v, s2); }
+            }
+        }
+        red[tid] = make_float2(s1, s2);
+        __syncthreads();
+        if (wid == 0) {
+            double d1 = 0.0, d2 = 0.0;
+#pragma unroll
+            for (int j = 0; j < 4; ++j) { const float2 v = red[lane + 64 * j]; d1 += (double)v.x; d2 += (double)v.y; }
+#pragma unroll
+            for (int o = 32; o >= 1; o >>= 1) {
+                d1 += __shfl_xor(d1, o, 64);
+                d2 += __shfl_xor(d2, o, 64);
+            }
+            if (lane == 0) {
+                double* dst = p.partials + ((size_t)b * p.ntiles + tile) * 2;
+                dst[0] = d1; dst[1] = d2;
+            }
+        }
+    }
+}
+int head_stats_ntiles(int T) { return ceil_div(T, HS_BN); }
+hipError_t launch_head_stats(const float* wav, const float* div, const float* w, double* partials, int B, int T, int padL, int padR, hipStream_t st) {
+    if (B < 1 || B > 65535 || T < 1 || padL < 0 || padR < 0 || padL + padR != RH_K1 - 1) return hipErrorInvalidValue;
+    HeadStatsArgs a;
+    a.wav = wav; a.div = div; a.w = w; a.partials = partials;
+    a.T = T; a.padL = padL; a.padR = padR;
+    const int maxpad = padL > padR ? padL : padR;
+    a.Leff = T > maxpad ? T : maxpad + 1;
+    a.ntiles = head_stats_ntiles(T);
+    hipLaunchKernelGGL(head_stats_kernel, dim3(a.ntiles < 4096 ? a.ntiles : 4096, B), dim3(256), 0, st, a);
+    return hipGetLastError();
 }
 
 __global__ __launch_bounds__(256) void gn_finalize_kernel(const double* __restrict__ partials, int nblk, double count,
diff --git a/funcodec_amd/engine.py b/funcodec_amd/engine.py
--- a/funcodec_amd/engine.py
+++ b/funcodec_amd/engine.py
@@ -560,6 +560,21 @@
         return y
 
     @_on_device
+    def debug_encoder_head(self, wav: torch.Tensor, scale: Optional[torch.Tensor], fold: bool):
+        wav = self._dev(wav, torch.float32)
+        B, T = wav.shape
+        scale = None if scale is None else self._dev(scale, torch.float32)
+        sc = torch.empty((B, 32, T), dtype=torch.float32, device=self.device)
+        b1 = torch.empty((B, 16, T), dtype=torch.float32, device=self.device)
+        nt = (T + 127) // 128
+        psc = torch.zeros((B, nt, 2), dtype=torch.float64, device=self.device)
+        pb1 = torch.zeros((B, nt, 2), dtype=torch.float64, device=self.device)
+        ws = self._scratch(B * 96 * (T + 64) * 4 + (4 << 20))
+        self._check(self.lib.fc_debug_encoder_head(self._h, _ptr(wav), _ptr(scale), B, T, 1 if fold else 0, _ptr(sc), _ptr(b1), _ptr(psc), _ptr(pb1),
+                                                   _ptr(ws), ws.numel(), self._stream()))
+        return sc, b1, psc, pb1
+
+    @_on_device
     def lstm_forward(self, prefix: str, x: torch.Tensor) -> torch.Tensor:
         x = self._dev(x, torch.float32)
         B, H, T = x.shape
diff --git a/include/funcodec_amd.h b/include/funcodec_amd.h
--- a/include/funcodec_amd.h
+++ b/include/funcodec_amd.h
@@ -177,6 +177,9 @@
                         float* y, void* workspace, size_t workspace_bytes, void* stream);
 int fc_resblock_forward_src(fc_engine* e, const char* prefix, const float* x0, const float* aff0, const float* x1, const float* aff1,
                             int B, int T, float* y, void* workspace, size_t workspace_bytes, void* stream);
+
+int fc_debug_encoder_head(fc_engine* e, const float* wav, const float* div, int B, int T, int fold, float* sc_raw, float* b1_raw,
+                          double* part_sc, double* part_b1, void* workspace, size_t workspace_bytes, void* stream);
 
 int fc_lstm_forward(fc_engine* e, const char* prefix, const float* x, int B, int T,
                     float* y, void* workspace, size_t workspace_bytes, void* stream);
```

Result: no change. 10750 audio-s/s (median of 6 runs) (+0.4%).
